# cage-challenge/cage-challenge-4

Hardware: AMD Instinct MI355X
Metric: agent-env steps/sec (5 blue agents x N envs) (higher is better)
Workload: dtype int32

## Files before the change

cage_challenge_4_amd/csrc/cc4_api.hip:

```cpp
#include "cc4_host.h"
#include "cc4_export.h"

static thread_local std::string g_create_err;
static std::mutex g_handles_mu;
static std::vector<cc4_handle*> g_handles;
std::atomic<int64_t> g_scoped_blocks{0};

__attribute__((constructor)) static void cc4_runtime_env() { setenv("GPU_MAX_HW_QUEUES", "16", 0); }

static int streams_run_concurrently(hipStream_t* st, int n) {
  if (n < 2) return 1;
  int khz = 100000, dev = 0;
  (void)hipGetDevice(&dev);
  (void)hipDeviceGetAttribute(&khz, hipDeviceAttributeWallClockRate, dev);
  if (khz <= 0) khz = 100000;
  const long long ticks = 300LL * khz / 1000;
  bool ok = true;
  double one = 0, all = 0;
  for (int pass = 0; pass < 2 && ok; ++pass) {
    const int m = pass ? n : 1;
    auto t0 = std::chrono::steady_clock::now();
    for (int i = 0; i < m; ++i) hipLaunchKernelGGL(k_spin, dim3(1), dim3(1), 0, st[i], ticks);
    for (int i = 0; i < m && ok; ++i) ok = hipStreamSynchronize(st[i]) == hipSuccess;
    const double us = std::chrono::duration<double, std::micro>(std::chrono::steady_clock::now() - t0).count();
    (pass ? all : one) = us;
  }
  return ok && all < 1.5 * (one > 300.0 ? one : 300.0);
}

static int policy_bits(const cc4_config& c) {
  return (c.red_policy & 3) | (c.green_policy ? GP_SLEEP_BIT : 0) | (c.green_policy == 2 ? GP_OPEN_BIT : 0) | (c.blue_policy ? BP_RANDOM_BIT : 0);
}
StepArgs step_args(const cc4_handle* h) {
  StepArgs a{};
  a.st = h->d_state; a.cold = h->d_cold;
  a.obs = h->d_obs; a.reward = h->d_reward; a.done = h->d_done; a.err = h->d_err;
  a.n = h->cfg.num_envs; a.autoreset = h->cfg.autoreset; a.steps = h->cfg.steps; a.rng_mode = h->cfg.rng_mode;
  a.policy = policy_bits(h->cfg);
  a.topo = (uint32_t)h->cfg.topology_seed;
  a.reset_ws = h->d_reset_ws;
  return a;
}
RunArgs run_args(const cc4_handle* h, int k, uint32_t t0, bool head) {
  RunArgs ra{};
  ra.progress = h->d_run; ra.slot_part = h->d_slot_part;
  ra.P = h->run_P; ra.K = k; ra.G = h->run_G; ra.t0 = t0;
  memcpy(ra.xcc_lo, h->xcc_lo, 8); memcpy(ra.xcc_n, h->xcc_n, 8);
  ra.thr = h->run_thr;
  ra.runs = head ? run_split_for_call(k, h->run_SA, h->run_SB, h->run_nB, h->run_single)
                 : run_split(k, h->run_SA, h->run_SB, h->run_nB, h->run_single);
  return ra;
}

void configure_groups(cc4_handle* h, int ng) {
  const int n = h->cfg.num_envs, cus = h->cus;
  if (ng < 1) ng = 1;
  if (ng > cc4_handle::MAX_GROUPS) ng = cc4_handle::MAX_GROUPS;
  if (ng > n) ng = n;
  h->ngroups = ng;
  for (int g = 0; g <= ng; ++g) h->glo[g] = (int)(((long long)n * g) / ng);
  const int gsize = (n + ng - 1) / ng;
  const int bpc = (gsize + cus - 1) / cus;
  const int bpc_all = (n + cus - 1) / cus;
  h->philox_minw = bpc <= 5 ? 1 : (bpc == 8 ? 8 : 7);
  if (ng > 1) h->philox_minw = bpc_all <= 6 ? 1 : 7;
  if (const char* v = getenv("CC4_PHILOX_MINW")) h->philox_minw = atoi(v);
  h->philox_lean = bpc > 8 || bpc_all > 13;
  if (const char* v = getenv("CC4_PHILOX_LEAN")) h->philox_lean = atoi(v) != 0;
}

int join_groups(cc4_handle* h) {
  if (h->rollout_k > 0 && !h->rollout_entering) { h->err = "a rollout is in flight on this handle: cc4_rollout_end first"; return -1; }
  if (h->ngroups > 1) {
    if (h->groups_busy) {
      for (int g = 1; g < h->ngroups; ++g) {
        HIPCHK(h, hipEventRecord(h->gev[g], h->gstream[g]));
        HIPCHK(h, hipStreamWaitEvent(h->stream, h->gev[g], 0));
      }
      h->groups_busy = false;
    }
    h->main_ahead = true;
    h->joined_between = true;
  }
  return 0;
}
int fork_groups(cc4_handle* h) {
  if (h->ngroups > 1 && h->main_ahead) {
    HIPCHK(h, hipEventRecord(h->mev, h->stream));
    for (int g = 1; g < h->ngroups; ++g) HIPCHK(h, hipStreamWaitEvent(h->gstream[g], h->mev, 0));
    h->main_ahead = false;
  }
  return 0;
}
int enter_refused(cc4_handle* h, const char* who, unsigned refuse) {
  if ((refuse & EN_NO_ROLLOUT) && h->rollout_k > 0) { h->err = std::string(who) + ": a rollout is in flight on this handle: cc4_rollout_end first"; return -2; }
  if ((refuse & EN_NO_COMM) && h->comm) { h->err = std::string(who) + ": not on a handle with a communicator"; return -2; }
  return 0;
}
int enter(cc4_handle* h, const char* who, unsigned refuse) {
  if (int rc = enter_refused(h, who, refuse)) return rc;
  HIPCHK(h, hipSetDevice(h->cfg.device_id));
  return join_groups(h) ? -1 : 0;
}
int copy_to_host(cc4_handle* h, const char* who, void* dst, const void* src, size_t bytes, hipMemcpyKind kind) {
  if (int rc = enter(h, who)) return rc;
  if (bytes) HIPCHK(h, hipMemcpyAsync(dst, src, bytes, kind, h->stream));
  HIPCHK(h, hipStreamSynchronize(h->stream));
  return 0;
}
int sync_all(cc4_handle* h) {
  for (int g = h->ngroups - 1; g >= 1; --g) if (h->groups_busy) HIPCHK(h, hipStreamSynchronize(h->gstream[g]));
  if (hipStreamQuery(h->stream) != hipSuccess) { (void)hipGetLastError(); HIPCHK(h, hipStreamSynchronize(h->stream)); }
  h->groups_busy = false;
  h->joined_between = true;
  return 0;
}

int wall_khz(cc4_handle* h) {
  if (h->khz <= 0) { int khz = 100000; (void)hipDeviceGetAttribute(&khz, hipDeviceAttributeWallClockRate, h->cfg.device_id); h->khz = khz > 0 ? khz : 100000; }
  return h->khz;
}
int ensure_watchdog_word(cc4_handle* h) {
  if (!h->h_xtimeout) {
// ... 91 lines not shown
const char* cc4_last_error(cc4_handle* h) { return h ? h->err.c_str() : g_create_err.c_str(); }
size_t cc4_state_bytes(void) { return sizeof(EnvState); }
int cc4_device_count(void) { int n = 0; return hipGetDeviceCount(&n) == hipSuccess ? n : 0; }
size_t cc4_algorithmic_bytes_per_env_step(void) {
  return 2 * sizeof(EnvState) + 4 * OBS_TOTAL + 4 * NBLUE + 4 + 1 + 4;
}
size_t cc4_hot_bytes(void) { return offsetof(EnvState, hd); }
const char* cc4_step_kernel(cc4_handle* h) {
  if (!h) return "";
  if (h->cfg.rng_mode != 1) return "k_step";
  return h->philox_lean ? "k_step_philox1" : "k_step_philox";
}

const char* cc4_run_kernel(cc4_handle* h) {
  if (!h) return "";
  const bool plain = (!h->comm || h->xchg_on) && !h->evlog_on && !h->ext_seen && !h->d_prof && !h->dbg_stop;
  if (plain && h->multistep) return h->multistep_minb == 8 ? "k_run_philox8" : "k_run_philox";
  if (plain && h->run1m) return "k_run_philox1m";
  if (plain && h->persist_state >= 0) return h->cfg.rng_mode == 0 ? "k_run_pcg" : (h->comm ? "k_run_philox1x" : "k_run_philox1");
  return cc4_step_kernel(h);
}
const char* cc4_run_kernel_for(cc4_handle* h, int32_t k) {
  if (!h) return "";
  if (h->persist_state == 0 && !h->run1m && !h->multistep && (!h->comm || h->xchg_on) && !h->evlog_on && !h->ext_seen && !h->d_prof && k >= h->persist_min_k && hipSetDevice(h->cfg.device_id) == hipSuccess) (void)persist_setup(h);
  const char* r = cc4_run_kernel(h);
  if (k < 2) return cc4_step_kernel(h);
  if (!h->multistep && !h->run1m && h->persist_state >= 0 && k < h->persist_min_k) return cc4_step_kernel(h);
  return r;
}

int cc4_create(const cc4_config* cfg, cc4_handle** out) {
  if (!cfg || !out || cfg->num_envs <= 0 || cfg->steps <= 0 || cfg->red_policy < 0 || cfg->red_policy > 3 ||
      cfg->green_policy < 0 || cfg->green_policy > 2 || cfg->blue_policy < 0 || cfg->blue_policy > 1 || cfg->rng_mode < 0 || cfg->rng_mode > 1) { g_create_err = "cc4_create: bad config"; return -2; }
  if (cfg->topology_seed != 0 && cfg->rng_mode != 1) { g_create_err = "cc4_create: topology_seed needs rng_mode 1 (the numpy stream draws scenario and dynamics from one generator)"; return -2; }
  int ndev = 0;
  hipError_t e = hipGetDeviceCount(&ndev);
  if (e != hipSuccess || ndev <= 0) {
    g_create_err = "cc4_create: no HIP device available (libcc4 has no CPU fallback)";
    return -3;
  }
  if (cfg->device_id < 0 || cfg->device_id >= ndev) { g_create_err = "cc4_create: device_id out of range"; return -2; }
  cc4_handle* h = new cc4_handle();
  h->cfg = *cfg;
  *out = h;
  { std::lock_guard<std::mutex> lk(g_handles_mu); g_handles.push_back(h); }
  if (const char* v = getenv("CC4_HOST_WAIT")) {
    static std::once_flag once;
    std::call_once(once, [v] {
      unsigned flags = hipDeviceScheduleAuto;
      if (!strcmp(v, "spin")) flags = hipDeviceScheduleSpin; else if (!strcmp(v, "yield")) flags = hipDeviceScheduleYield; else if (!strcmp(v, "block")) flags = hipDeviceScheduleBlockingSync;
      (void)hipSetDeviceFlags(flags);
      (void)hipGetLastError();
    });
  }
  HIPCHK(h, hipSetDevice(cfg->device_id));
  if (cc4_upload_pcg_tables() != hipSuccess) { h->err = "cc4_create: the numpy-stream kernel's jump table could not be uploaded"; return -1; }
  {
    hipDeviceProp_t prop;
    HIPCHK(h, hipGetDeviceProperties(&prop, cfg->device_id));
    h->cus = prop.multiProcessorCount > 0 ? prop.multiProcessorCount : 256;
  }
  {
    int ng = cfg->num_envs >= 1024 ? 3 : (cfg->num_envs >= 512 ? 2 : 1);
    h->auto_groups = getenv("CC4_GROUPS") == nullptr;
    if (const char* v = getenv("CC4_GROUPS")) ng = atoi(v);
    configure_groups(h, ng);
  }
  if (new_stream(h, &h->stream)) return -1;
  h->gstream[0] = h->stream;
  for (int g = 1; g < h->ngroups; ++g) {
    if (new_stream(h, &h->gstream[g]) || new_event(h, &h->gev[g], hipEventDisableTiming)) return -1;
  }
  if (new_event(h, &h->mev, hipEventDisableTiming) || new_event(h, &h->ev_wait, hipEventDisableTiming) || new_event(h, &h->ev_signal, hipEventDisableTiming)) return -1;
  if (h->auto_groups && h->ngroups == 3) {
    if (new_stream(h, &h->gstream[3])) return -1;
    if (streams_run_concurrently(h->gstream, 4)) {
      if (new_event(h, &h->gev[3], hipEventDisableTiming)) return -1;
      configure_groups(h, 4);
    } else release(h, &h->gstream[3]);
  }
  size_t n = (size_t)cfg->num_envs;
  h->cold_row = cold_row_bytes(cfg->steps);
  if (dev_alloc(h, &h->d_state, n * sizeof(EnvState)) || dev_alloc(h, &h->d_cold, n * h->cold_row)) return -1;
  if (dev_alloc(h, &h->d_reset_ws, cfg->rng_mode == 1 ? n * RESET_WS_WORDS * sizeof(uint32_t) : n * 128 * sizeof(uint64_t))) return -1;
  h->in_bytes = n * NBLUE * sizeof(int32_t) + n * NBLUE * MSG_LEN;
  h->small_io = cfg->num_envs <= cc4_handle::SMALL_IO_ENVS;
  if (const char* v = getenv("CC4_SMALL_IO")) h->small_io = h->small_io && atoi(v) != 0;
  if (h->small_io) {
    if (pin_alloc(h, &h->pin_in, h->in_bytes)) return -1;
    HIPCHK(h, hipHostGetDevicePointer(reinterpret_cast<void**>(&h->d_actions), h->pin_in, 0));
    memset(h->pin_in, 0, h->in_bytes);
  } else if (dev_alloc(h, &h->d_actions, h->in_bytes)) return -1;
  h->d_msgs = reinterpret_cast<uint8_t*>(h->d_actions) + n * NBLUE * sizeof(int32_t);
  if (dev_alloc(h, &h->d_seeds, n * sizeof(uint64_t)) || dev_alloc(h, &h->d_envmask, n)) return -1;
  h->out_bytes = n * OBS_TOTAL * sizeof(int32_t) + n * sizeof(float) + n * sizeof(uint32_t) + n;
  if (h->small_io) {
    if (pin_alloc(h, &h->pin_out, h->out_bytes)) return -1;
    HIPCHK(h, hipHostGetDevicePointer(reinterpret_cast<void**>(&h->d_obs), h->pin_out, 0));
  } else if (dev_alloc(h, &h->d_obs, h->out_bytes)) return -1;
  h->d_reward = reinterpret_cast<float*>(h->d_obs + n * OBS_TOTAL);
  h->d_err = reinterpret_cast<uint32_t*>(h->d_reward + n);
  h->d_done = reinterpret_cast<uint8_t*>(h->d_err + n);
  if (dev_alloc(h, &h->d_mask, n * MASK_TOTAL) || dev_alloc(h, &h->d_rng, n * 7 * sizeof(uint64_t))) return -1;
  if (dev_alloc(h, &h->d_claim, n * sizeof(uint32_t) + sizeof(uint32_t)) || dev_alloc(h, &h->d_mask_stale, n)) return -1;
  h->d_copy_fault = h->d_claim + n;
  HIPCHK(h, hipMemsetAsync(h->d_claim, 0, n * sizeof(uint32_t) + sizeof(uint32_t), h->stream));
  HIPCHK(h, hipMemsetAsync(h->d_mask_stale, 0, n, h->stream));
  HIPCHK(h, hipMemsetAsync(h->d_state, 0, n * sizeof(EnvState), h->stream));
  HIPCHK(h, hipMemsetAsync(h->d_cold, 0, n * h->cold_row, h->stream));
  HIPCHK(h, hipMemsetAsync(h->d_obs, 0, n * OBS_TOTAL * sizeof(int32_t), h->stream));
  HIPCHK(h, hipMemsetAsync(h->d_done, 0, n, h->stream));
  HIPCHK(h, hipMemsetAsync(h->d_err, 0, n * sizeof(uint32_t), h->stream));
  HIPCHK(h, hipStreamSynchronize(h->stream));
  if (choose_run_form(h, 0)) return -1;
  if (const char* v = getenv("CC4_PERSIST_MIN_K")) h->persist_min_k = atoi(v);
  if (const char* v = getenv("CC4_WHOLE_BATCH_STEPS")) h->whole_batch_steps = atoi(v) != 0;
  if (const char* v = getenv("CC4_PERSIST_VERIFY")) h->verify = atoi(v) != 0;
  if (const char* v = getenv("CC4_PERSIST_VERIFY_EVERY")) h->verify_every = atoi(v) > 0 ? atoi(v) : 0;
  return 0;
}

void cc4_destroy(cc4_handle* h) {
  if (!h) return;
  enq_pool_stop(h);
  (void)hipSetDevice(h->cfg.device_id);
  for (const OwnedList::Entry& e : h->own.entries) if (e.kind == OWN_STREAM && *e.field) (void)hipStreamSynchronize(static_cast<hipStream_t>(*e.field));
  if (h->comm) ncclCommDestroy(h->comm);
  if (h->shadow) { cc4_destroy(h->shadow); h->shadow = nullptr; (void)hipSetDevice(h->cfg.device_id); }
  h->own.release_all();
  { std::lock_guard<std::mutex> lk(g_handles_mu); g_handles.erase(std::remove(g_handles.begin(), g_handles.end(), h), g_handles.end()); }
  delete h;
}
int cc4_debug_live_resources(int64_t out[4]) {
  if (!out) return -2;
  out[OWN_DEVICE] = g_scoped_blocks.load(); out[OWN_PINNED] = out[OWN_EVENT] = out[OWN_STREAM] = 0;
  std::lock_guard<std::mutex> lk(g_handles_mu);
  for (const cc4_handle* h : g_handles) h->own.count_live(out);
  return 0;
}

static int reset_launch(cc4_handle* h, const uint64_t* d_seeds, const uint8_t* d_env_mask) {
  ResetArgs a{h->d_state, h->d_cold, d_seeds, d_env_mask, h->d_obs, h->d_reward,
              h->d_done, h->d_err, h->d_mask, h->cfg.num_envs, h->cfg.steps, h->cfg.rng_mode,
              policy_bits(h->cfg), (uint32_t)h->cfg.topology_seed,
              h->comm ? h->d_obs8[h->obs_buf] : nullptr};
  if (h->comm && h->gathers_issued > h->gathers_waited) { HIPCHK(h, hipStreamSynchronize(h->comm_stream)); h->gathers_waited = h->gathers_issued; }
  if (h->comm && h->obs8_from_slab >= 0) {
    const size_t row = (size_t)h->cfg.num_envs * OBS_PACKED;
    if (d_env_mask) HIPCHK(h, hipMemcpyAsync(h->d_obs8[h->obs_buf], h->d_xslab + (size_t)h->obs8_from_slab * row, row, hipMemcpyDeviceToDevice, h->stream));
    h->obs8_from_slab = -1;
  }
  hipLaunchKernelGGL(k_reset, dim3(h->cfg.num_envs), dim3(WAVE), 0, h->stream, a);
  HIPCHK(h, hipGetLastError());
  h->prev_valid = false;
  h->step_event_attached = false;
  return 0;
}
int cc4_reset(cc4_handle* h, const uint64_t* seeds, const uint8_t* env_mask) {
  if (int rc = enter(h, "cc4_reset")) return rc;
  size_t n = (size_t)h->cfg.num_envs;
  if (seeds) HIPCHK(h, hipMemcpyAsync(h->d_seeds, seeds, n * sizeof(uint64_t), hipMemcpyHostToDevice, h->stream));
  if (env_mask) HIPCHK(h, hipMemcpyAsync(h->d_envmask, env_mask, n, hipMemcpyHostToDevice, h->stream));
  if (int rc = reset_launch(h, seeds ? h->d_seeds : nullptr, env_mask ? h->d_envmask : nullptr)) return rc;
  HIPCHK(h, hipStreamSynchronize(h->stream));
  return 0;
}
int cc4_reset_device(cc4_handle* h, const uint64_t* d_seeds, const uint8_t* d_env_mask) {
// ... 505 lines not shown
```

cage_challenge_4_amd/csrc/cc4_api_debug.hip:

```cpp
#include "cc4_host.h"

int timeline_report(cc4_handle* h, int k, bool timed) {
  std::vector<unsigned long long> tl(4 * (size_t)h->run_grid);
  HIPCHK(h, hipMemcpy(tl.data(), h->d_timeline, tl.size() * sizeof(unsigned long long), hipMemcpyDeviceToHost));
  release(h, &h->d_timeline);
#ifdef CC4_BOUNDARY_PROF
  { double sA = 0, sB = 0, sC = 0, sD = 0, sn = 0, items = 0, busy_ticks = 0; int nw = 0; std::vector<double> per;
    bool head = false;
    for (int w = 0; w < h->run_grid; ++w) { const unsigned long long* t = &tl[4 * (size_t)w]; if (!(t[0] >> 63)) continue; head = true;
      const double n = (double)((t[0] >> 32) & 0x7FFFFFFFull); if (n <= 0) continue; ++nw;
      const double A = (double)(uint32_t)t[1], B = (double)(t[1] >> 32), C = (double)(uint32_t)t[2], D = (double)(t[2] >> 32);
      sA += A; sB += B; sC += C; sD += D; sn += n; items += (double)(uint32_t)t[3]; busy_ticks += (double)(uint32_t)t[0]; per.push_back((A + B + C + D) / n / 100.0); }
    if (head) {
      float ms = 0.f; if (timed) (void)hipEventElapsedTime(&ms, h->evs[0], h->evs[1]);
      std::sort(per.begin(), per.end());
      const size_t m = per.size();
      const RunSplit rs = h->last_runs;
      if (m) fprintf(stderr, "[cc4 boundary] k=%d runs SA=%d nA=%d SB=%d nB=%d nph=%d: %d waves with a boundary, %.0f boundaries (%.0f items); per boundary, mean us: stage-out drain + publish %.3f, pick %.3f, "
                      "progress wait + acquire %.3f, stage-in %.3f, all %.3f; per wave all: min %.3f / median %.3f / 90%% %.3f / max %.3f us; boundaries are %.2f %% of the waves' busy time "
                      "(first item's start to last item's end, mean %.1f us); kernel (events) %.1f us\n", k, rs.SA, rs.nA, rs.SB, rs.nB, rs.nph, nw, sn, items,
                      sA / sn / 100.0, sB / sn / 100.0, sC / sn / 100.0, sD / sn / 100.0, (sA + sB + sC + sD) / sn / 100.0, per[0], per[m / 2], per[m * 9 / 10], per[m - 1],
                      100.0 * (sA + sB + sC + sD) / busy_ticks, busy_ticks / nw / 100.0, ms * 1000.0);
      return 0;
    }
  }
#endif
  unsigned long long e0 = ~0ull, e1 = 0, f1 = 0, l0 = ~0ull, l1 = 0; double fs = 0, ls = 0, items = 0; int nw = 0, idle = 0;
  for (int w = 0; w < h->run_grid; ++w) { const unsigned long long* t = &tl[4 * (size_t)w]; if (!t[0]) continue; ++nw; e0 = t[0] < e0 ? t[0] : e0; e1 = t[0] > e1 ? t[0] : e1; if (!(uint32_t)t[3]) { ++idle; continue; } f1 = t[1] > f1 ? t[1] : f1; l0 = t[2] < l0 ? t[2] : l0; l1 = t[2] > l1 ? t[2] : l1; fs += (double)t[1]; ls += (double)t[2]; items += (double)(uint32_t)t[3]; }
  const int busy = nw - idle;
  float ms = 0.f; if (timed) (void)hipEventElapsedTime(&ms, h->evs[0], h->evs[1]);
  fprintf(stderr, "[cc4 timeline] k=%d: %d waves reported (%d without an item); entry spread %.1f us; first item starts: mean +%.1f us, last +%.1f us after the first entry; "
                  "last item ends: earliest +%.1f us, mean +%.1f us, latest +%.1f us; items per busy wave %.1f; kernel (events) %.1f us\n",
          k, nw, idle, (e1 - e0) / 100.0, busy ? (fs / busy - (double)e0) / 100.0 : 0.0, (f1 - e0) / 100.0, (l0 - e0) / 100.0, busy ? (ls / busy - (double)e0) / 100.0 : 0.0, (l1 - e0) / 100.0, busy ? items / busy : 0.0, ms * 1000.0);
  { std::map<int, std::pair<unsigned long long, double>> cu;
    for (int w = 0; w < h->run_grid; ++w) { const unsigned long long* t = &tl[4 * (size_t)w]; if (!t[0] || !(uint32_t)t[3]) continue; auto& c = cu[(int)((t[3] >> 32) - 1)]; if (t[2] > c.first) c.first = t[2]; c.second += (double)(uint32_t)t[3]; }
    std::vector<double> last, its; for (auto& kv : cu) { last.push_back((kv.second.first - e0) / 100.0); its.push_back(kv.second.second); }
    std::sort(last.begin(), last.end()); std::sort(its.begin(), its.end());
    if (!last.empty()) { const size_t m = last.size(); fprintf(stderr, "[cc4 timeline]   per CU (%zu): last wave dry at min %.1f / 10%% %.1f / median %.1f / 90%% %.1f / max %.1f us; items executed min %.0f / median %.0f / max %.0f\n", m,
                               last[0], last[m / 10], last[m / 2], last[m * 9 / 10], last[m - 1], its[0], its[m / 2], its[m - 1]); } }
  { double xs[8] = {0}, xi[8] = {0}; unsigned long long xl[8] = {0}, xf[8]; int xn[8] = {0}; for (int i = 0; i < 8; ++i) xf[i] = ~0ull;
    for (int w = 0; w < h->run_grid; ++w) { const unsigned long long* t = &tl[4 * (size_t)w]; if (!t[0] || !(uint32_t)t[3]) continue; const int xc = (int)(((t[3] >> 32) - 1) >> 8) & 7;
      xs[xc] += (double)t[2]; xi[xc] += (double)(uint32_t)t[3]; ++xn[xc]; if (t[2] > xl[xc]) xl[xc] = t[2]; if (t[2] < xf[xc]) xf[xc] = t[2]; }
    for (int i = 0; i < 8; ++i) if (xn[i]) fprintf(stderr, "[cc4 timeline]   XCD %d: %d busy waves, %.0f items; waves ran dry: earliest +%.1f, mean +%.1f, latest +%.1f us\n", i, xn[i], xi[i],
                                                  (xf[i] - e0) / 100.0, (xs[i] / xn[i] - (double)e0) / 100.0, (xl[i] - e0) / 100.0); }
  return 0;
}
void exchange_prof_report(int k, const std::chrono::steady_clock::time_point (&t)[6]) {
  static double xp[6] = {0}; static long xpn = 0;
  auto us = [](std::chrono::steady_clock::time_point a, std::chrono::steady_clock::time_point b) { return std::chrono::duration<double, std::micro>(b - a).count(); };
  xp[0] += us(t[0], t[1]); xp[1] += us(t[1], t[2]); xp[2] += us(t[2], t[3]); xp[3] += us(t[3], t[4]); xp[4] += us(t[4], t[5]); xp[5] += us(t[0], t[5]);
  if (++xpn % 200 == 0) {
    fprintf(stderr, "[cc4 exchange prof] k=%d, mean of 200 calls (us): begin %.1f, launch %.1f, enqueue of the chunks %.1f, wait for the kernel %.1f, then for the communication stream %.1f; call %.1f\n",
            k, xp[0] / 200, xp[1] / 200, xp[2] / 200, xp[3] / 200, xp[4] / 200, xp[5] / 200);
    for (double& v : xp) v = 0;
  }
}
int cc4_debug_rollout_state(cc4_handle* h, int64_t* out ) {
  if (!h->d_rcnt) { h->err = "cc4_debug_rollout_state: no rollout was begun on this handle"; return -2; }
  HIPCHK(h, hipSetDevice(h->cfg.device_id));
  std::vector<uint32_t> rd(32), cnt((size_t)h->run_P * RPG_MAX * cc4_handle::XRING);
  uint32_t fail = 0;
  HIPCHK(h, hipMemcpy(rd.data(), h->d_rready, rd.size() * 4, hipMemcpyDeviceToHost));
  HIPCHK(h, hipMemcpy(cnt.data(), h->d_rcnt, cnt.size() * 4, hipMemcpyDeviceToHost));
  HIPCHK(h, hipMemcpy(&fail, h->d_rfail, 4, hipMemcpyDeviceToHost));
  out[0] = fail; out[1] = *reinterpret_cast<volatile uint32_t*>(h->h_xtimeout);
  for (int g = 0; g < h->rpg; ++g) out[2 + g] = rd[g];
  for (int slot = 0; slot < 4; ++slot) for (int g = 0; g < h->rpg; ++g) {
    int64_t sum = 0;
    for (int p = 0; p < h->run_P; ++p) sum += cnt[((size_t)p * h->rpg + g) * cc4_handle::XRING + slot];
    out[6 + 4 * slot + g] = sum;
  }
  return 0;
}

int cc4_debug_profile(cc4_handle* h, int enable, unsigned long long* out) {
  if (int rc = enter(h, "cc4_debug_profile")) return rc;
  size_t bytes = (size_t)h->cfg.num_envs * PROF_SLOTS * sizeof(unsigned long long);
  if (enable && !h->d_prof) { if (dev_alloc(h, &h->d_prof, bytes)) return -1; HIPCHK(h, hipMemsetAsync(h->d_prof, 0, bytes, h->stream)); }
  if (out && h->d_prof) { HIPCHK(h, hipMemcpyAsync(out, h->d_prof, bytes, hipMemcpyDeviceToHost, h->stream)); HIPCHK(h, hipStreamSynchronize(h->stream)); }
  if (!enable) release(h, &h->d_prof);
  return 0;
}

int cc4_debug_stop_phase(cc4_handle* h, int phase) {
  if (join_groups(h)) return -1;
  if (phase < 0 || phase > 14 || !h->philox_lean) { h->err = "cc4_debug_stop_phase: phase 0..14, on a handle whose step kernel is k_step_philox1"; return -2; }
  h->dbg_stop = phase;
  return 0;
}

int cc4_debug_persist_base(cc4_handle* h, uint32_t base) {
  if (h->rollout_k > 0) { h->err = "cc4_debug_persist_base: a rollout is in flight on this handle"; return -2; }
  if (base > PROGRESS_CLEAR_AT) { char msg[64]; snprintf(msg, sizeof msg, "cc4_debug_persist_base: base 0 .. %#x", PROGRESS_CLEAR_AT); h->err = msg; return -2; }
  if (int rc = enter(h, "cc4_debug_persist_base")) return rc;
  if (h->persist_state == 0) { if (persist_setup(h)) return -1; }
  if (h->persist_state != 1) { h->err = "cc4_debug_persist_base: this handle has no persistent kernel"; return -2; }
  HIPCHK(h, hipMemsetD32Async(reinterpret_cast<hipDeviceptr_t>(h->d_run), (int)base, (size_t)h->cfg.num_envs, h->stream));
  HIPCHK(h, hipStreamSynchronize(h->stream));
  h->pool_base = base;
  return 0;
}
int cc4_debug_copy_from_device(cc4_handle* h, void* host_dst, const void* device_src, size_t bytes) {
  if (int rc = enter(h, "cc4_debug_copy_from_device")) return rc;
  HIPCHK(h, hipStreamSynchronize(h->stream));
  for (int g = 0; g < 4; ++g) if (h->gpolicy[g]) HIPCHK(h, hipStreamSynchronize(h->gpolicy[g]));
// ... 58 lines not shown
```

cage_challenge_4_amd/csrc/cc4_args.h:

```cpp
#pragma once
#include <hip/hip_runtime.h>

#include "../../include/cc4.h"
#include "cc4_engine.h"
#include "cc4_sched.h"

using namespace cc4;

static_assert(sizeof(EnvState) % 16 == 0 && offsetof(EnvState, hd) % 16 == 0, "EnvState rows are staged with 16-byte accesses");
constexpr int ROW_VEC = (int)(sizeof(EnvState) / 16);
constexpr int HOT_VEC = (int)(offsetof(EnvState, hd) / 16);
constexpr int WAVE = 64;
constexpr int OBS_PACKED = CC4_OBS_PACKED_BYTES;
static_assert(OBS_PACKED % 4 == 0 && OBS_PACKED * 4 >= OBS_TOTAL, "packed observation row: whole words, four values per byte");
constexpr int PROF_SLOTS = 128;

constexpr int cc4_handle_max_groups = 8;

#ifndef CC4_PERSIST_MINW
#define CC4_PERSIST_MINW 6
#endif
#ifndef CC4_LEAN_MINW
#define CC4_LEAN_MINW 1
#endif
#ifndef CC4_SMALL_MINW
#define CC4_SMALL_MINW 1
#endif
#ifndef CC4_PHILOX_BIG_MINW
#define CC4_PHILOX_BIG_MINW 7
#endif

struct StepArgs {
  EnvState* st; EnvCold* cold;
  const int32_t* actions; const uint8_t* msgs;
  int32_t* obs; float* reward; uint8_t* done; uint32_t* err;
  uint8_t* obs8;
  int32_t* rand_out;
  uint64_t rand_seed0; uint32_t rand_t;
  int n, autoreset, steps, rng_mode, policy;
  int full_obs;
  uint32_t topo;
  unsigned long long* prof;
  uint32_t* reset_ws;
  const ExtAct* ext;
  int e0;
  int act_sys;
  int dbg_stop;
};

struct XchgArgs {
  uint8_t* slab;
  uint32_t* gathered;
  uint32_t* timeout;
  int ring;
  long long wait_ticks;
  uint32_t* gcnt;
  uint32_t* timeout_host;
};

struct RunArgs {
  uint32_t* progress;
  const int32_t* slot_part;
  int P, K;
  int G;
  uint32_t t0;
  RunSplit runs;
  uint8_t xcc_lo[8], xcc_n[8];
  int thr;
  uint32_t* ticket;
  uint32_t* ticket_next;
  uint32_t base;
  unsigned long long* timeline;
  const uint32_t* act_ready;
  const int32_t* act;
  int PG;
  long long act_wait_ticks;
};
constexpr int TK_STRIDE = 32;
constexpr int CC4_SLOTS = 2048;
constexpr int RPG_MAX = 4;

struct PlanArgs {
  const int32_t* actions;
  const uint8_t* msgs;
  float* rewards;
  uint8_t* dones;
  uint8_t* obs_packed;
  uint32_t* err_or;
};
constexpr uint32_t PLAN_REGEN = 0x80000000u;

struct ResetArgs {
  EnvState* st; EnvCold* cold; const uint64_t* seeds; const uint8_t* env_mask;
  int32_t* obs; float* reward; uint8_t* done; uint32_t* err; uint8_t* mask;
  int n, steps, rng_mode, policy;
  uint32_t topo;
  uint8_t* obs8;
};

struct alignas(16) SlotHdr {
  uint32_t magic, version;
  int32_t steps, rng_mode;
  uint32_t claim;
  uint32_t pad[11];
};
static_assert(sizeof(SlotHdr) == 64, "64-byte slot header");
constexpr uint32_t SLOT_MAGIC = 0x45344343u;
constexpr uint32_t SLOT_VERSION = (1u << 24) | (uint32_t)((sizeof(EnvState) + sizeof(EnvCold)) & 0xFFFFFFu);
constexpr size_t SLOT_OUT_BYTES = 192;
CC4_HD size_t slot_cold_off() { return sizeof(SlotHdr) + sizeof(EnvState); }
CC4_HD size_t slot_out_off(size_t cold_row) { return slot_cold_off() + ((cold_row + 63) & ~(size_t)63); }
CC4_HD size_t slot_bytes(size_t cold_row) { return slot_out_off(cold_row) + SLOT_OUT_BYTES; }
static_assert(OBS_PACKED + 12 <= (int)SLOT_OUT_BYTES && sizeof(SlotHdr) % 64 == 0 && sizeof(EnvState) % 64 == 0, "slot layout");
enum : uint32_t { CF_RANGE = CC4_COPY_RANGE, CF_DUP_DST = CC4_COPY_DUP_DST, CF_SRC_IS_DST = CC4_COPY_SRC_IS_DST, CF_SLOT_EMPTY = CC4_COPY_SLOT_EMPTY,
                  CF_SLOT_CONFIG = CC4_COPY_SLOT_CONFIG };
CC4_HD uint32_t slot_hdr_fault(const SlotHdr* hdr, int steps, int rng_mode) {
  if (hdr->magic != SLOT_MAGIC || hdr->version != SLOT_VERSION) return CF_SLOT_EMPTY;
  return hdr->steps != steps || hdr->rng_mode != rng_mode ? CF_SLOT_CONFIG : 0u;
}
struct CopyArgs {
  EnvState* st; EnvCold* cold; size_t cold_row;
  int32_t* obs; float* reward; uint8_t* done; uint32_t* err; uint8_t* mask; uint8_t* mask_stale;
  uint32_t* claim;
  const uint8_t* src_bank; uint8_t* dst_bank; size_t slot;
  const int32_t* src; const int32_t* dst; const uint64_t* seeds;
  int count, n, src_cap, dst_cap, steps, rng_mode, evlog_on;
// ... 56 lines not shown
```

cage_challenge_4_amd/csrc/cc4_engine.h:

```cpp
#pragma once
#include "cc4_state.h"
#include "cc4_tables.h"

namespace cc4 {

struct Ctx { EnvState* s; EnvCold* c; Rng* r; HostDyn* hd; StepWork* w; unsigned long long* prof = nullptr;
             unsigned long long* aprof = nullptr; EvLog* lg = nullptr; const uint64_t* gpre = nullptr;
             const ExtAct* ext = nullptr; };

#if defined(__HIP_DEVICE_COMPILE__)
#define CC4_TICK(x, i) do { if ((x).prof) { unsigned long long _t = clock64(); (x).prof[(i)] += _t - (x).prof[15]; (x).prof[15] = _t; } } while (0)
#define CC4_TICK0(x) do { if ((x).prof) (x).prof[15] = clock64(); } while (0)
#define CC4_AT0(x) unsigned long long _at = (x).aprof ? clock64() : 0
#define CC4_AT(x, k) do { if ((x).aprof) { unsigned long long _n = clock64(); (x).aprof[(k)] += _n - _at; _at = _n; } } while (0)
#if defined(CC4_FINE)
#define CC4_FT0(x, r) unsigned long long _ft = ((x).aprof && (r) == 0) ? clock64() : 0
#define CC4_FT(x, r, k) do { if ((x).aprof && (r) == 0) { unsigned long long _n = clock64(); (x).aprof[88 + (k)] += _n - _ft; _ft = _n; } } while (0)
#else
#define CC4_FT0(x, r) do { } while (0)
#define CC4_FT(x, r, k) do { } while (0)
#endif
#else
#define CC4_FT0(x, r) do { } while (0)
#define CC4_FT(x, r, k) do { } while (0)
// ... 524 lines not shown
  if (flags & OE_SYSHN) bit_set(a.as_hn, host);
  if (subnet_known) a.h.as_subnet |= (uint16_t)(1u << h_subnet(host));
  uint8_t want = (uint8_t)(key_ip ? OE_KEY_IP : 0);
  uint32_t* has = a.obs_has[key_ip ? 1 : 0];
  if (bit_get(has, host)) {
    for (int i = 0; i < a.h.nobs; ++i)
      if (a.obs[i].host == host && (a.obs[i].flags & OE_KEY_IP) == want) { a.obs[i].flags |= (uint8_t)flags; return; }
  }
  bit_set(has, host);
  if (a.h.nobs >= MAX_OBS) { set_err(x, E_OBS_OVERFLOW); return; }
  a.obs[a.h.nobs].host = (uint8_t)host;
  a.obs[a.h.nobs].flags = (uint8_t)(flags | want);
  a.h.nobs++;
}
CC4_HD void obs_first(Ctx x, int r, int success, int atype, int ahost, int aarg) {
  RedAgent& a = x.s->red[r];
  if (a.h.obs_success != 0) return;
  const uint32_t v = hdr_obs_word((uint32_t)success, (uint32_t)atype, (uint32_t)ahost, (uint32_t)aarg);
  __builtin_memcpy(__builtin_assume_aligned(reinterpret_cast<char*>(&a.h) + offsetof(RedHdr, obs_success), 4), &v, 4);
}

CC4_HD int path_to_root(int h, uint8_t* out) {
  int n = 0;
  out[n++] = (uint8_t)h;
  if (h == H_INTERNET) return n;
  int s = h_subnet(h);
  if (!h_is_router(h)) out[n++] = (uint8_t)h_make(s, 0);
  while (true) {
    int p = router_parent(s);
    if (p == S_INT) { out[n++] = (uint8_t)H_INTERNET; break; }
    out[n++] = (uint8_t)h_make(p, 0);
    s = p;
  }
  return n;
}
CC4_HD int route(int src, int dst, uint8_t* work) {
  uint8_t* a = work; uint8_t* b = work + 6; uint8_t* out = work + 12;
  int na = path_to_root(src, a), nb = path_to_root(dst, b);
  while (na >= 2 && nb >= 2 && a[na - 2] == b[nb - 2]) { na--; nb--; }
  int n = 0;
  for (int i = 0; i < na; ++i) out[n++] = a[i];
  for (int i = nb - 2; i >= 0; --i) out[n++] = b[i];
  return n;
}

CC4_HD int gen_pid(Ctx x, uint32_t* used) {
  while (true) {
    int pid = rng_range(x.r, 1000, 10000);
    if (!bit_get(used, pid - 1000)) { bit_set(used, pid - 1000); return pid; }
  }
}
CC4_HD int start_session_proc(Ctx x, int h, int kind) {
  HostDyn& st = x.hd[h];
  int mx = 0;
  for (int i = 0; i < st.nproc; ++i) if (st.procs[i].pid > mx) mx = st.procs[i].pid;
  int pid = mx + 1 + (int)rng_below(x.r, 9);
  st.procs[st.nproc].pid = (uint16_t)pid; st.procs[st.nproc].kind = (uint8_t)kind; st.procs[st.nproc].flags = 0;
  st.nproc++;
  return pid;
}
CC4_HD void host_backup(Ctx x, int h, int ip_octet) {
  const HostDyn& d = x.hd[h];
  HostStatic st;
  for (int i = 0; i < 8; ++i) st.procs[i] = d.procs[i];
  for (int i = 0; i < 5; ++i) st.svcs[i] = d.svcs[i];
  st.nproc = (uint8_t)d.nproc; st.nsvc = (uint8_t)hd_nsvc(d); st.exists = (uint8_t)(1 | ((d.gtmp & 1) << 1)); st.ip_octet = (uint8_t)ip_octet;
  if (d.nproc > PIN - 1 || hd_nsvc(d) > 5) set_err(x, E_PROC_OVERFLOW);
  __builtin_memcpy(&x.c->hs[h], &st, sizeof(HostStatic));
}
CC4_HD void host_restore(Ctx x, int h) {
  hd_touch(x, h);
  HostDyn& d = x.hd[h];
  HostStatic st;
  __builtin_memcpy(&st, &x.c->hs[h], sizeof(HostStatic));
  for (int i = 0; i < 8; ++i) d.procs[i] = st.procs[i];
  for (int i = 0; i < 5; ++i) d.svcs[i] = st.svcs[i];
  d.nproc = st.nproc; d.gtmp = 0; d.nsf = st.nsvc;
  x.s->hev[h] = 0;
  eph_clear(x, h);
  pend_drop_host(x, h);
}

struct ResetCarry { uint64_t env_key; };
enum : int { RESET_WS_SEEN = 0, RESET_WS_DUP = 288, RESET_WS_HOSTS = 576, RESET_WS_WORDS = 584 };

CC4_HD void reset_zero(EnvState* s, HostDyn* hd, EnvCold* c, int t, int nt) {
  static_assert(offsetof(EnvState, rng) == 0, "the generator leads the row");
  uint32_t* w = (uint32_t*)s;
  for (size_t i = sizeof(Rng) / 4 + (size_t)t; i < offsetof(EnvState, hd) / 4; i += (size_t)nt) w[i] = i == PA_WORD ? w[i] & PA_WORD_MASK : 0;
  uint32_t* hw = (uint32_t*)hd;
  for (size_t i = (size_t)t; i < sizeof(HostDyn) * MAXH / 4; i += (size_t)nt) hw[i] = 0;
  uint32_t* b = (uint32_t*)c->hs;
  for (size_t i = (size_t)t; i < sizeof(c->hs) / 4; i += (size_t)nt) b[i] = 0;
}
static_assert(sizeof(RSess) * RS_POOL >= 4 * 282, "the idle session pool holds the 9000-bit pid set of the generation");
CC4_HD uint32_t* reset_used_set(EnvState* s) { return reinterpret_cast<uint32_t*>(s->spool); }
CC4_HD void reset_used_clear(EnvState* s, int t, int nt) { uint32_t* u = reset_used_set(s); for (int i = t; i < 282; i += nt) u[i] = 0; }
template <int RNG_MODE>
CC4_HD void reset_gen_host(Ctx x, int h) {
  EnvState* s = x.s;
  if (!bit_get(s->exists, h)) return;
  if (RNG_MODE == 1) rng_set_stream(x.r, ST_GEN_HOST + (uint32_t)h);
  HostDyn& st = x.hd[h];
  st.gtmp = (uint8_t)rng_below(x.r, 2);
  if (h_is_router(h)) return;
  int n = 0;
  auto put = [&](int kind, int pid) {
    st.svcs[n].kind = (uint8_t)kind; st.svcs[n].pid = (uint16_t)pid; st.svcs[n].st = (uint8_t)(SV_ACTIVE | 5);
    st.procs[n].kind = (uint8_t)kind; st.procs[n].pid = (uint16_t)pid; st.procs[n].flags = 0;
    n++;
  };
  auto pid = [&]() { return RNG_MODE == 1 ? rng_range(x.r, 1000, 10000) : gen_pid(x, reset_used_set(s)); };
  put(K_SSHD, pid());
  int sub = h_subnet(h);
  if (sub == S_OZA || sub == S_OZB) put(K_OT, pid());
  int p_apache = pid(), p_mysql = pid(), p_smtp = pid();
  int n_add = (int)rng_below(x.r, 4);
  uint32_t left = 7;
  for (int k = 0; k < n_add; ++k) {
    int o = nth_bit(left, (int)rng_below(x.r, (uint32_t)popc32(left)));
    left &= ~(1u << o);
    put(o == 0 ? K_APACHE : (o == 1 ? K_MYSQL : K_SMTP), o == 0 ? p_apache : (o == 1 ? p_mysql : p_smtp));
  }
  for (int i = 0; i < n; ++i) (void)rng_random(x.r);
  hd_set_nsvc(st, n); st.nproc = (uint16_t)n;
  if (RNG_MODE == 1) { st.procs[5].pid = (uint16_t)p_apache; st.procs[6].pid = (uint16_t)p_mysql; st.svcs[6].pid = (uint16_t)p_smtp; }
}
struct ResetHostLater { CC4_HD void operator()(Ctx, int) const {} };
struct ResetHostNow { CC4_HD void operator()(Ctx x, int h) const { reset_gen_host<0>(x, h); } };
CC4_HD void reset_mission_phases(EnvState* s, int steps) {
  int q = steps / 3, rem = steps % 3;
  s->steps = steps;
  s->phase_len[0] = q + (rem >= 1 ? 1 : 0); s->phase_len[1] = q + (rem == 2 ? 1 : 0); s->phase_len[2] = q;
}
template <int RNG_MODE, typename HostHook>
CC4_HD ResetCarry reset_topology(Ctx x, uint64_t seed, int steps, bool continue_stream, int policy, uint32_t topo_seed, uint32_t* ws,
                                 bool rng_is_copy, HostHook host_placed) {
  EnvState* s = x.s;
  if (!continue_stream) rng_seed(&s->rng, seed, (uint32_t)RNG_MODE);
  s->rng_mode = (uint8_t)RNG_MODE;
  s->policy = (uint8_t)policy_at_reset(s, policy);
  rng_begin_episode(x.r);
  ResetCarry k; k.env_key = x.r->s_lo;
  if (RNG_MODE == 1 && topo_seed) x.r->s_lo = (uint64_t)topo_seed;
  reset_mission_phases(s, steps);
  if (RNG_MODE == 1) for (int i = 0; i < RESET_WS_WORDS; ++i) ws[i] = 0;
  {
    uint32_t* avail = x.w->scratch;
    for (int i = 0; i < 8; ++i) avail[i] = 0xFFFFFFFFu;
    int n = 256;
    for (int sn = 0; sn < NSUB; ++sn) {
      int v = nth_set(avail, 8, (int)rng_below(x.r, (uint32_t)n));
      s->cidr_octet[sn] = (uint8_t)v;
      bit_clr(avail, v);
      n--;
    }
  }
  for (int sn = 0; sn < NSUB; ++sn) {
    uint32_t* ips = x.w->scratch;
    for (int i = 0; i < 8; ++i) ips[i] = 0xFFFFFFFFu;
    ips[0] &= ~1u; ips[7] &= 0x7FFFFFFFu;
    int n = 254;
    auto place = [&](int h, int v) {
      bit_clr(ips, v); n--; bit_set(s->exists, h); x.hd[h].procs[PIN - 1].pid = (uint16_t)v;
      host_placed(x, h);
    };
    if (sn == S_INT) { place(H_INTERNET, nth_set(ips, 8, (int)rng_below(x.r, (uint32_t)n))); continue; }
    place(h_make(sn, 0), nth_set(ips, 8, (int)rng_below(x.r, (uint32_t)n)));
    int nu = 3 + (int)rng_below(x.r, 8);
    for (int i = 0; i < nu; ++i) place(h_make(sn, 1 + i), nth_set(ips, 8, (int)rng_below(x.r, (uint32_t)n)));
    int ns = 1 + (int)rng_below(x.r, 6);
    for (int i = 0; i < ns; ++i) place(h_make(sn, 11 + i), last_set(ips, 8));
    s->n_users[sn] = (uint8_t)nu; s->n_servers[sn] = (uint8_t)ns;
  }
  if (RNG_MODE == 1 && rng_is_copy) s->rng = *x.r;
  return k;
}
CC4_HD void reset_pid_serial(Ctx x, uint32_t* used) {
  EnvState* s = x.s;
  for (int h = 0; h < MAXH; ++h) {
    if (!bit_get(s->exists, h) || h_is_router(h)) continue;
    HostDyn& st = x.hd[h];
    const int n = hd_nsvc(st);
    const int sub = h_subnet(h);
    const int nfix = (sub == S_OZA || sub == S_OZB) ? 2 : 1;
    Rng t; bool forked = false;
    auto settle = [&](int v0, bool* moved) {
      int v = v0 - 1000;
      *moved = false;
      while (bit_get(used, v)) {
        if (!forked) { rng_fork(&t, x.r, ST_GEN_REDRAW + (uint32_t)h); forked = true; }
        v = (int)rng_below(&t, 9000);
        *moved = true;
      }
      bit_set(used, v);
      return v + 1000;
    };
    for (int i = 0; i < nfix; ++i) {
      bool moved;
      const int v = settle(st.svcs[i].pid, &moved);
      if (moved) { st.svcs[i].pid = (uint16_t)v; st.procs[i].pid = (uint16_t)v; }
    }
    for (int k = 0; k < 3; ++k) {
      const int kind = k == 0 ? K_APACHE : (k == 1 ? K_MYSQL : K_SMTP);
      const int v0 = k == 0 ? st.procs[5].pid : (k == 1 ? st.procs[6].pid : st.svcs[6].pid);
      bool moved;
      const int v = settle(v0, &moved);
      if (moved) for (int i = nfix; i < n; ++i) if (st.svcs[i].kind == kind) { st.svcs[i].pid = (uint16_t)v; st.procs[i].pid = (uint16_t)v; }
    }
    st.procs[5].pid = 0; st.procs[6].pid = 0; st.svcs[6].pid = 0;
  }
}
CC4_HD void reset_agents(Ctx x) {
  EnvState* s = x.s;
  for (int b = 0; b < NBLUE; ++b) {
    int nsub = blue_nsub(b);
    (void)rng_below(x.r, (uint32_t)nsub);
    int cnt = 0;
    for (int i = 0; i < nsub; ++i) { int sn = blue_subnet_alloc(b, i); cnt += 1 + s->n_users[sn] + s->n_servers[sn]; }
    int c = (int)rng_below(x.r, (uint32_t)cnt);
    int ph = -1;
    for (int i = 0; i < nsub && ph < 0; ++i) {
      int sn = blue_subnet_alloc(b, i), nu = s->n_users[sn], ns = s->n_servers[sn];
      if (c < 1 + nu) ph = h_make(sn, c);
      else if (c < 1 + nu + ns) ph = h_make(sn, 11 + (c - 1 - nu));
      else c -= 1 + nu + ns;
    }
    s->blue[b].parent_host = (uint8_t)ph;
  }
  {
    int g = 0;
    for (int sn = 0; sn < NSUB - 1; ++sn) for (int i = 0; i < s->n_users[sn]; ++i) s->green_host[g++] = (uint8_t)h_make(sn, 1 + i);
    s->n_green = (uint8_t)g;
  }
  for (int r = 0; r < NRED; ++r) {
    int sn = red_subnet_alloc(r, (int)rng_below(x.r, (uint32_t)red_nsub(r)));
    int c = (int)rng_below(x.r, (uint32_t)(s->n_users[sn] + s->n_servers[sn]));
    s->red[r].h.start_host = (uint8_t)(c < s->n_users[sn] ? h_make(sn, 1 + c) : h_make(sn, 11 + (c - s->n_users[sn])));
    s->red[r].h.new_sess_host = 0xFF;
  }
}
CC4_HD void reset_seal_host(Ctx x, int h) {
  host_backup(x, h, x.hd[h].procs[PIN - 1].pid);
  x.hd[h].procs[PIN - 1].pid = 0; x.hd[h].gtmp = 0;
}
CC4_HD void reset_host_sessions(Ctx x, int h) {
  EnvState* s = x.s;
  if (!bit_get(s->exists, h)) return;
  rng_set_stream(x.r, ST_GEN_SESS + (uint32_t)h);
  if (blue_of_subnet(h_subnet(h)) >= 0) (void)start_session_proc(x, h, K_SESS_BLUE);
  if (h != H_INTERNET && h_is_user(h)) (void)start_session_proc(x, h, K_SESS_GREEN);
  if (h == s->red[0].h.start_host) (void)start_session_proc(x, h, K_SESS_RED);
  reset_seal_host(x, h);
}
CC4_HD void reset_sessions_agent_order(Ctx x) {
  EnvState* s = x.s;
  for (int b = 0; b < NBLUE; ++b) {
    int ph = s->blue[b].parent_host;
    (void)start_session_proc(x, ph, K_SESS_BLUE);
    for (int i = 0; i < blue_nsub(b); ++i) {
      int sn = blue_subnet_alloc(b, i);
      for (int sl = 0; sl < SLOTS; ++sl) {
        int h = h_make(sn, sl);
        if (!bit_get(s->exists, h) || h == ph) continue;
        (void)start_session_proc(x, h, K_SESS_BLUE);
      }
    }
  }
  for (int g = 0; g < s->n_green; ++g) (void)start_session_proc(x, s->green_host[g], K_SESS_GREEN);
  (void)start_session_proc(x, s->red[0].h.start_host, K_SESS_RED);
}
CC4_HD void reset_seal_all_hosts(Ctx x) {
  EnvState* s = x.s;
  for (int h = 0; h < MAXH; ++h) {
    if (bit_get(s->exists, h)) reset_seal_host(x, h);
    eph_clear(x, h);
  }
  s->npend = 0;
}
CC4_HD void reset_finish(Ctx x, ResetCarry k, int steps, uint32_t topo_seed, bool rng_is_copy) {
  EnvState* s = x.s;
  {
    const HostDyn& d = x.hd[s->red[0].h.start_host];
    int red0_pid = 0;
    for (int i = 0; i < d.nproc; ++i) if (d.procs[i].kind == K_SESS_RED) red0_pid = d.procs[i].pid;
    (void)rs_add(x, 0, s->red[0].h.start_host, red0_pid, RS_ABSTRACT | RS_ORIG);
    s->red[0].h.active = 1;
  }
  for (int r = 0; r < NRED; ++r) {
    RedAgent& a = s->red[r];
    int h = a.h.start_host;
    bit_set(a.as_ip, h); bit_set(a.as_hn, h); a.h.as_subnet |= (uint16_t)(1u << h_subnet(h));
    if (r == 0) {
      as_know_sid(x, 0, 0);
      obs_put(x, 0, false, h, OE_SESS | OE_IFACE | OE_SYSHN, true);
      obs_first(x, 0, T_UNKNOWN, RA_NONE, 0, 0);
    }
    a.h.exec_type = RA_SLEEP;
  }
  s->done = (uint8_t)(0 >= steps - 1);
  s->n_actions = NBLUE + s->n_green + NRED;
  x.c->rwd = RewardRec{};
  if (topo_seed) x.r->s_lo = k.env_key;
  if (rng_is_copy) s->rng = *x.r;
  rng_park(&s->rng);
}
CC4_HD void env_reset_counter_mode(Ctx x, uint64_t seed, int steps, bool continue_stream, int policy, uint32_t topo_seed, uint32_t* ws,
                                   bool rng_is_copy) {
  reset_zero(x.s, x.hd, x.c, 0, 1);
  ResetCarry k = reset_topology<1>(x, seed, steps, continue_stream, policy, topo_seed, ws, rng_is_copy, ResetHostLater{});
  {
    Rng t; rng_fork(&t, x.r, ST_GEN_HOST);
    Ctx xh = x; xh.r = &t;
    for (int h = 0; h < MAXH; ++h) reset_gen_host<1>(xh, h);
  }
  reset_pid_serial(x, reset_used_set(x.s));
  reset_used_clear(x.s, 0, 1);
  reset_agents(x);
  {
    Rng t; rng_fork(&t, x.r, ST_GEN_SESS);
    Ctx xh = x; xh.r = &t;
    for (int h = 0; h < MAXH; ++h) reset_host_sessions(xh, h);
  }
  reset_finish(x, k, steps, topo_seed, rng_is_copy);
}
CC4_HD void env_reset_numpy_stream(Ctx x, uint64_t seed, int steps, bool continue_stream, int policy, bool rng_is_copy) {
  reset_zero(x.s, x.hd, x.c, 0, 1);
  ResetCarry k = reset_topology<0>(x, seed, steps, continue_stream, policy, 0, nullptr, rng_is_copy, ResetHostNow{});
  reset_used_clear(x.s, 0, 1);
  reset_agents(x);
  reset_sessions_agent_order(x);
  reset_seal_all_hosts(x);
  reset_finish(x, k, steps, 0, rng_is_copy);
}

CC4_HD void env_reset(Ctx x, uint64_t seed, int rng_mode, int steps, bool continue_stream, int policy = 0, uint32_t topo_seed = 0,
                      uint32_t* ws = nullptr, bool rng_is_copy = false) {
  if (rng_mode == 1) env_reset_counter_mode(x, seed, steps, continue_stream, policy, topo_seed, ws, rng_is_copy);
  else env_reset_numpy_stream(x, seed, steps, continue_stream, policy, rng_is_copy);
}

enum : int { BLUE_RAW_ACTION = 0x10000 };
CC4_HD constexpr uint32_t blue_slot_shape(int b, int idx) {
  const int nsub = blue_nsub(b), nh = ZONE_HOSTS * nsub, nc = 8 * nsub;
  int t = BA_SLEEP, j = 0;
  if (idx < 0 || idx >= 4 * nh + 2 + 2 * nc) return (uint32_t)BA_SLEEP;
  if (idx < nh) { t = BA_ANALYSE; j = idx; }
  else if (idx == nh) return (uint32_t)BA_MONITOR;
  else if (idx < 2 * nh + 1) { t = BA_REMOVE; j = idx - nh - 1; }
  else if (idx < 3 * nh + 1) { t = BA_RESTORE; j = idx - 2 * nh - 1; }
  else if (idx == 3 * nh + 1) return (uint32_t)BA_SLEEP;
  else if (idx < 3 * nh + 2 + nc) { t = BA_ALLOW; j = idx - 3 * nh - 2; }
  else if (idx < 3 * nh + 2 + 2 * nc) { t = BA_BLOCK; j = idx - 3 * nh - 2 - nc; }
  else { t = BA_DECOY; j = idx - 3 * nh - 2 - 2 * nc; }
  if (t == BA_ALLOW || t == BA_BLOCK) {
    const int dst = blue_subnet_sorted(b, j / 8), k = j % 8;
    int src = 0, c = 0;
    for (int i = 0; i < NSUB; ++i) { const int sn = sorted_subnet(i); if (sn == dst) continue; if (c == k) { src = sn; break; } c++; }
    return (uint32_t)t | ((uint32_t)dst << 8) | ((uint32_t)src << 16);
  }
  const int sn = blue_subnet_sorted(b, j / ZONE_HOSTS), hs = j % ZONE_HOSTS;
  const int h = hs < MAX_SERVERS ? h_make(sn, 11 + hs) : h_make(sn, 1 + (hs - MAX_SERVERS));
  return (uint32_t)t | ((uint32_t)h << 8);
}
#if defined(__HIP_DEVICE_COMPILE__)
struct BlueSlotTab { uint32_t v[NBLUE][ACT_LONG]; };
constexpr BlueSlotTab make_blue_slot_tab() {
  BlueSlotTab t{};
  for (int b = 0; b < NBLUE; ++b) for (int i = 0; i < ACT_LONG; ++i) t.v[b][i] = blue_slot_shape(b, i);
  return t;
}
static __device__ const BlueSlotTab blue_slot_tab = make_blue_slot_tab();
__device__ __forceinline__ uint32_t blue_slot(int b, int idx) { return blue_slot_tab.v[b][idx]; }
#else
CC4_HD uint32_t blue_slot(int b, int idx) { return blue_slot_shape(b, idx); }
#endif
CC4_HD Act blue_decode(const EnvState* s, int b, int idx) {
  Act a; a.type = BA_SLEEP; a.host = 0; a.arg = 0; a.ticks = 1; a.sid = 0; a.busy = 0;
  int nsub = blue_nsub(b), nh = ZONE_HOSTS * nsub, nc = 8 * nsub;
  int total = 4 * nh + 2 + 2 * nc;
  if (idx >= BLUE_RAW_ACTION) {
    const int t = (idx >> 8) & 0xF, h = idx & 0xFF;
    if (t == BA_BLOCK || t == BA_ALLOW) {
      const int to = h & 0xF, from = h >> 4;
      if (to >= NSUB || from >= NSUB) return a;
      a.type = (uint8_t)t; a.host = (uint8_t)to; a.arg = (uint8_t)from;
      return a;
    }
    if (t == BA_MONITOR) { a.type = BA_MONITOR; return a; }
    if (t < BA_ANALYSE || t > BA_DECOY || h >= H_INTERNET || !bit_get(s->exists, h) || blue_of_subnet(h_subnet(h)) != b) return a;
    a.type = (uint8_t)t; a.host = (uint8_t)h;
    return a;
  }
  if (idx < 0 || idx >= total) return a;
  const uint32_t sh = blue_slot(b, idx);
  const int t = (int)(sh & 0xFF), h = (int)((sh >> 8) & 0xFF);
  if (t == BA_SLEEP) return a;
  if (t == BA_MONITOR) { a.type = BA_MONITOR; return a; }
  if (t == BA_ALLOW || t == BA_BLOCK) { a.type = (uint8_t)t; a.host = (uint8_t)h; a.arg = (uint8_t)(sh >> 16); return a; }
// ... 1621 lines not shown
```

cage_challenge_4_amd/csrc/cc4_host.h:

```cpp
#pragma once
#include <hip/hip_runtime.h>
#include <hip/hip_ext.h>
#include <rccl/rccl.h>
#include <stdio.h>
#include <stdlib.h>
#include <string.h>
#include <string>
#include <chrono>
#include <vector>
#include <deque>
#include <map>
#include <algorithm>
#include <thread>
#include <mutex>
#include <condition_variable>
#include <atomic>

#include "../../include/cc4_debug.h"
#include "cc4_args.h"
#include "cc4_kernel_decls.h"
#include "cc4_export.h"
#include "cc4_digest.h"
#include "cc4_owned.h"
#define CC4_HOST __attribute__((visibility("hidden")))

inline void free_device(void* p) { (void)hipFree(p); }
inline void free_pinned(void* p) { (void)hipHostFree(p); }
inline void free_event(void* p) { (void)hipEventDestroy(static_cast<hipEvent_t>(p)); }
inline void free_stream(void* p) { (void)hipStreamDestroy(static_cast<hipStream_t>(p)); }

struct cc4_handle {
  cc4_config cfg;
  OwnedList own{{free_device, free_pinned, free_event, free_stream}, {}};
  hipStream_t stream = nullptr;
  EnvState* d_state = nullptr; EnvCold* d_cold = nullptr;
  size_t cold_row = 0;
  int32_t* d_actions = nullptr; uint8_t* d_msgs = nullptr; uint64_t* d_seeds = nullptr; uint8_t* d_envmask = nullptr;
  int32_t* d_obs = nullptr; float* d_reward = nullptr; uint8_t* d_done = nullptr; uint32_t* d_err = nullptr;
  uint8_t* d_mask = nullptr; uint64_t* d_rng = nullptr;
  size_t out_bytes = 0, in_bytes = 0;
  uint8_t* pin_out = nullptr; uint8_t* pin_in = nullptr;
  static constexpr int SMALL_IO_ENVS = 16;
  bool small_io = false;
  bool keep_prev = false, prev_valid = false;
  EnvState* d_prev_state = nullptr; EnvCold* d_prev_cold = nullptr; uint8_t* d_prev_out = nullptr;
  const int32_t* prev_actions = nullptr; const uint8_t* prev_msgs = nullptr; bool prev_full_obs = false, prev_ext = false;
  static constexpr int OBS_RING = 8, OBS_WAIT_EVERY = 4;
  static constexpr int MAX_GROUPS = cc4_handle_max_groups;
  uint8_t* d_obs8[OBS_RING] = {};
  uint8_t* d_all_obs8[OBS_RING] = {};
  long long gather_seq[OBS_RING] = {};
  long long gathers_issued = 0, gathers_waited = 0;
  hipEvent_t tev_start[cc4_handle_max_groups] = {}, tev_stop[cc4_handle_max_groups] = {};
  long long comm_delay_ticks = 0;
  long long gather_stalls = 0;
  long long stat_steps = 0; double stat_launch_us = 0, stat_gather_us = 0;
  hipStream_t comm_stream = nullptr;
  hipEvent_t ev_step[OBS_RING][MAX_GROUPS] = {}, ev_comm[OBS_RING] = {};
  int obs_buf = 0;
  int gather_buf = -1;
  bool step_event_attached = false;
  int ngroups = 1;
  int cus = 256;
  int glo[MAX_GROUPS + 1] = {};
  hipStream_t gstream[MAX_GROUPS] = {};
  hipEvent_t gev[MAX_GROUPS] = {};
  hipEvent_t mev = nullptr;
  hipEvent_t ev_wait = nullptr, ev_signal = nullptr;
  bool auto_groups = true;
  bool groups_busy = false;
  bool joined_between = false;
  bool main_ahead = false;
  unsigned long long* d_prof = nullptr;
  int dbg_stop = 0;
  uint32_t* d_reset_ws = nullptr;
  uint8_t* d_unpacked = nullptr;
  int evlog_on = 0;
  uint32_t* d_run = nullptr;
  int32_t* d_slot_part = nullptr;
  unsigned long long* d_timeline = nullptr;
  size_t run_words = 0;
  int run_P = 0, run_grid = 0;
  int run_G = 0;
  uint8_t xcc_lo[8] = {0}, xcc_n[8] = {0};
  int run_thr = 16;
  uint32_t* d_pool = nullptr;
  int run_SA = 0, run_SB = 1, run_nB = 0, run_single = 0;
  RunSplit last_runs{};
  uint32_t pool_base = 0;
  int pool_parity = 0;
  int persist_state = -1;
  bool whole_batch_steps = true;
  int run_margin = 0;
  static constexpr int XRING = 32;
  bool xchg_on = false;
  int xchg_chunk = 8;
  uint8_t* d_xslab = nullptr;
  uint8_t* d_xall = nullptr;
  int khz = 0;
  int32_t* d_ract = nullptr;
  uint32_t* d_rready = nullptr;
  uint32_t* d_rcnt = nullptr;
  uint32_t* d_rfail = nullptr;
  hipStream_t policy_stream = nullptr;
  hipStream_t gpolicy[4] = {nullptr, nullptr, nullptr, nullptr};
  hipEvent_t rev = nullptr;
  int rollout_k = 0;
  bool rollout_entering = false;
  int rollout_watchdog_ms = 2000;
  int rollout_margin = 1;
  int rpg = 4;
  int obs8_from_slab = -1;
  uint32_t* d_xflags = nullptr;
  uint32_t* d_xgcnt = nullptr;
  uint32_t* h_xtimeout = nullptr;
  uint32_t* d_xtimeout = nullptr;
  int xflags_clean = 0;
  hipEvent_t xev = nullptr;
  long long xchg_calls = 0, xchg_timeouts = 0;
  int xchg_watchdog_ms = 2000;
  uint8_t* last_gathered = nullptr;
  uint8_t* d_xlog = nullptr;
  int xlog_cap = 0, xlog_n = 0;
  bool persist_refused = false;
  bool verify = false, is_shadow = false;
  int verify_every = 1024;
  uint64_t persist_calls = 0;
  cc4_handle* shadow = nullptr;
  uint64_t* d_digest = nullptr;
  uint32_t* d_plan_err = nullptr;
  long long verify_calls = 0, verify_mismatches = 0;
  struct VerifyPlant { int32_t part = -1, env = 0, step = 0; int64_t offset = 0; } plant;
  int persist_min_k = 10;
  struct EnqPool* pool = nullptr;
  bool enq_threads = false;
  bool run1m = false;
  int multistep_minb = 5;
  bool multistep = false;
  ExtAct* d_ext = nullptr;
  bool ext_seen = false, ext_dirty = false;
  bool ext_submitted = false, terms_on = false;
  bool ext_green_dirty = true;
  std::vector<ExtAct> h_ext;
  bool full_obs_next = true;
  uint32_t full_obs_gmask = 0;
  bool philox_lean = false;
  int philox_minw = 1;
  ncclComm_t comm = nullptr; int rank = 0, world = 1;
  uint32_t* d_claim = nullptr; uint32_t* d_copy_fault = nullptr; uint8_t* d_mask_stale = nullptr;
  int32_t* d_copy_idx = nullptr; uint64_t* d_copy_seeds = nullptr;
  int8_t* d_pol = nullptr;
  std::deque<hipEvent_t> evs;
  std::string err;
};

#define HIPCHK(h, call)                                                                        \
  do {                                                                                         \
    hipError_t _e = (call);                                                                    \
// ... 79 lines not shown
```

cage_challenge_4_amd/csrc/cc4_k_misc.hip:

```cpp
#include "cc4_persist.h"
#include "cc4_kernel_decls.h"
#include "cc4_digest.h"

__global__ __launch_bounds__(WAVE) void k_xchg_gate(uint32_t* gcnt, int ring, int groups, int n, int P, int k_lo, int k_hi, long long ticks, uint32_t* fail, int max_naps) {
  const int t = (int)threadIdx.x, steps = k_hi - k_lo + 1;
  const long long t0 = wall_clock64();
  for (int i = t; i < groups * steps; i += (int)blockDim.x) {
    const int g = i / steps, k = k_lo + i % steps;
    const int size = P > 0 ? part_episodes(n, P, g) : xchg_group32_size(n, g);
    if (size <= 0) continue;
    uint32_t* c = gcnt + (size_t)g * (size_t)ring + (k % ring);
    int naps = 1;
    while (__hip_atomic_load(c, __ATOMIC_RELAXED, __HIP_MEMORY_SCOPE_AGENT) < (uint32_t)size) {
      for (int q = 0; q < naps; ++q) __builtin_amdgcn_s_sleep(127);
      if (naps < max_naps) naps <<= 1;
      if (wall_clock64() - t0 > ticks) { __hip_atomic_store(fail, 1u, __ATOMIC_RELAXED, __HIP_MEMORY_SCOPE_SYSTEM); break; }
    }
    __hip_atomic_store(c, 0u, __ATOMIC_RELAXED, __HIP_MEMORY_SCOPE_AGENT);
  }
}
__global__ __launch_bounds__(WAVE) void k_discover(int32_t* count, long long ticks) {
  if (threadIdx.x == 0) {
    atomicAdd(&count[cu_slot()], 1);
    const long long t0 = wall_clock64();
    while (wall_clock64() - t0 < ticks) __builtin_amdgcn_s_sleep(32);
  }
}
__global__ __launch_bounds__(WAVE) void k_reset(ResetArgs a) {
  __shared__ uint8_t obs_lds[OBS_TOTAL + 2];
  __shared__ uint8_t mask_lds[MASK_TOTAL + 2];
  __shared__ StepWork work;
  const int e = blockIdx.x, lane = threadIdx.x;
  if (e >= a.n) return;
  if (a.env_mask && !a.env_mask[e]) return;
  EnvCold* const cold_e = cold_at(a.cold, (size_t)e, cold_row_bytes(a.steps));
  EnvState* s = a.st + e;
  HostDyn* const hd = s->hd;
  for (int i = lane; i < (int)(sizeof(StepWork) / 4); i += WAVE) reinterpret_cast<uint32_t*>(&work)[i] = 0;
  __syncthreads();
  if (a.rng_mode == 1) {
    __shared__ uint32_t ws[RESET_WS_WORDS];
    reset_counter_mode_block<WAVE, false>(s, hd, cold_e, &work, lane, ws, a.seeds ? a.seeds[e] : 0, a.seeds == nullptr, a.steps, a.policy, a.topo);
    __syncthreads();
  } else if (lane == 0) {
    Ctx x{s, cold_e, &s->rng, hd, &work};
    env_reset(x, a.seeds ? a.seeds[e] : 0, 0, a.steps, a.seeds == nullptr, a.policy, a.topo);
  }
  if (lane == 0) {
    env_flat_obs<uint8_t>(s, obs_lds);
    blue_action_mask(s, mask_lds);
    a.reward[e] = 0.f; a.done[e] = s->done; a.err[e] = s->err;
  }
  __syncthreads();
  int32_t* o = a.obs + (size_t)e * OBS_TOTAL;
  for (int i = lane; i < OBS_TOTAL; i += WAVE) o[i] = obs_lds[i];
  uint8_t* m = a.mask + (size_t)e * MASK_TOTAL;
  for (int i = lane; i < MASK_TOTAL; i += WAVE) m[i] = mask_lds[i];
  if (a.obs8) store_packed_row(a.obs8 + (size_t)e * OBS_PACKED, obs_lds, lane, WAVE);
}

__global__ void k_random_actions(int32_t* actions, int n, uint64_t seed0, uint32_t t, int e0) {
  int i = e0 * NBLUE + blockIdx.x * blockDim.x + threadIdx.x;
  if (i >= n * NBLUE) return;
  int e = i / NBLUE, b = i % NBLUE;
  actions[i] = random_blue_action(seed0, t, e, b);
}

__global__ void k_spin(long long cycles) {
  const long long t0 = wall_clock64();
  while (wall_clock64() - t0 < cycles) __builtin_amdgcn_s_sleep(32);
}

__global__ void k_unpack_obs(const uint8_t* __restrict__ packed, uint8_t* __restrict__ out, int rows) {
  const int r = blockIdx.x, j = threadIdx.x;
  if (r >= rows || j >= OBS_PACKED) return;
  const uint32_t b = packed[(size_t)r * OBS_PACKED + j];
  uint8_t* o = out + (size_t)r * OBS_TOTAL + 4 * j;
#pragma unroll
  for (int k = 0; k < 4; ++k) if (4 * j + k < OBS_TOTAL) o[k] = (uint8_t)((b >> (2 * k)) & 3u);
}

template <int DT> __device__ __forceinline__ uint32_t policy_half_bits(int x) {
  constexpr uint64_t tab = DT == 1 ? 0x420040003C000000ull : 0x404040003F800000ull;
  return (uint32_t)(tab >> (16 * (x & 3))) & 0xFFFFu;
}
template <int DT> __device__ __forceinline__ void policy_obs_put(void* out, size_t i, int4 v) {
  if constexpr (DT == 0) {
    reinterpret_cast<uint32_t*>(out)[i] = (uint32_t)(v.x & 0xFF) | (uint32_t)(v.y & 0xFF) << 8 | (uint32_t)(v.z & 0xFF) << 16 | (uint32_t)(v.w & 0xFF) << 24;
  } else if constexpr (DT == 3) {
    reinterpret_cast<float4*>(out)[i] = make_float4((float)v.x, (float)v.y, (float)v.z, (float)v.w);
  } else {
    reinterpret_cast<uint2*>(out)[i] = make_uint2(policy_half_bits<DT>(v.x) | policy_half_bits<DT>(v.y) << 16, policy_half_bits<DT>(v.z) | policy_half_bits<DT>(v.w) << 16);
  }
}
template <int DT> __device__ __forceinline__ void policy_obs_part(const int32_t* __restrict__ obs, void* __restrict__ out, size_t total, size_t i0, size_t stride) {
  const size_t nv = total / 4;
  const int4* __restrict__ src = reinterpret_cast<const int4*>(obs);
  for (size_t i = i0; i < nv; i += stride) policy_obs_put<DT>(out, i, src[i]);
  if (i0 == 0) {
    for (size_t j = 4 * nv; j < total; ++j) {
      const int x = obs[j];
      if constexpr (DT == 0) reinterpret_cast<uint8_t*>(out)[j] = (uint8_t)x;
      else if constexpr (DT == 3) reinterpret_cast<float*>(out)[j] = (float)x;
      else reinterpret_cast<uint16_t*>(out)[j] = (uint16_t)policy_half_bits<DT>(x);
    }
  }
}
__global__ __launch_bounds__(256) void k_policy_outputs(const EnvState* __restrict__ st, const int32_t* __restrict__ obs, const float* __restrict__ reward,
                                                        const uint8_t* __restrict__ done, const uint32_t* __restrict__ err, int n, int ep_blocks, int dtype,
                                                        void* __restrict__ out_obs, uint8_t* __restrict__ out_mask, float* __restrict__ out_reward,
                                                        uint8_t* __restrict__ out_done, int32_t* __restrict__ out_err, uint8_t* __restrict__ mask_stale) {
  if ((int)blockIdx.x < ep_blocks) {
    const int e = (int)(blockIdx.x * blockDim.x + threadIdx.x), lane = (int)threadIdx.x & (WAVE - 1);
    bool regen = false;
    if (e < n) {
      out_reward[e] = reward[e]; out_done[e] = done[e]; out_err[e] = (int32_t)err[e];
      regen = st[e].step_count == 0;
      if (mask_stale[e]) { regen = true; mask_stale[e] = 0; }
    }
    unsigned long long todo = __ballot(regen);
    while (todo) {
      const int k = __ffsll(todo) - 1;
      todo &= todo - 1;
      const int er = e - lane + k;
      const EnvState* s = st + er;
// ... 129 lines not shown
```

cage_challenge_4_amd/csrc/cc4_k_pcg.hip:

```cpp
#include "cc4_kernels.h"
#include "cc4_persist.h"

struct PcgJump { uint64_t a_hi, a_lo, b_hi, b_lo; };
__device__ PcgJump g_pcg_jump[WAVE + 1];
__device__ __forceinline__ uint64_t bcast64(uint64_t v) {
  return (uint64_t)(uint32_t)__builtin_amdgcn_readfirstlane((int)(uint32_t)v) | ((uint64_t)(uint32_t)__builtin_amdgcn_readfirstlane((int)(uint32_t)(v >> 32)) << 32);
}
__device__ __forceinline__ uint32_t rdlane(uint32_t v, int j) { return (uint32_t)__builtin_amdgcn_readlane((int)v, j); }
__device__ __forceinline__ uint64_t lane64(uint64_t v, int src) {
  return (uint64_t)(uint32_t)__builtin_amdgcn_readlane((int)(uint32_t)v, src) | ((uint64_t)(uint32_t)__builtin_amdgcn_readlane((int)(uint32_t)(v >> 32), src) << 32);
}
__device__ __forceinline__ void pcg_ahead(const PcgJump& J, uint64_t s_hi, uint64_t s_lo, uint64_t i_hi, uint64_t i_lo, uint64_t* o_hi, uint64_t* o_lo) {
  const uint64_t p_lo = J.a_lo * s_lo, p_hi = __umul64hi(J.a_lo, s_lo) + J.a_hi * s_lo + J.a_lo * s_hi;
  const uint64_t q_lo = J.b_lo * i_lo, q_hi = __umul64hi(J.b_lo, i_lo) + J.b_hi * i_lo + J.b_lo * i_hi;
  const uint64_t lo = p_lo + q_lo;
  *o_lo = lo; *o_hi = p_hi + q_hi + (lo < p_lo ? 1ull : 0ull);
}
__device__ __forceinline__ uint64_t pcg_output(uint64_t hi, uint64_t lo) {
  const uint64_t v = hi ^ lo; const uint32_t rot = (uint32_t)(hi >> 58);
  return (v >> rot) | (v << ((64u - rot) & 63u));
}
__device__ __forceinline__ bool wave_green_policy(Rng& rl, int n, uint8_t* green_act, int lane) {
  const uint64_t s_hi = bcast64(rl.s_hi), s_lo = bcast64(rl.s_lo), i_hi = bcast64(rl.inc_hi), i_lo = bcast64(rl.inc_lo);
  const uint32_t has32 = (uint32_t)__builtin_amdgcn_readfirstlane((int)rl.has32), u32 = (uint32_t)__builtin_amdgcn_readfirstlane((int)rl.u32);
// ... 191 lines not shown
      int i = 0; uint32_t n32 = 0; bool hard = false;
      auto fetch = [&]() { uint64_t v = f[0]; if (i == 1) v = f[1]; if (i == 2) v = f[2]; if (i == 3) v = f[3]; if (i >= 4) v = f[4]; ++i; return v; };
      auto take32 = [&]() { ++n32; if (has) { has = 0; return buf; } const uint64_t o = fetch(); buf = (uint32_t)(o >> 32); q_new = pos + i - 1; has = 1; return (uint32_t)o; };
      auto below = [&](uint32_t n) { if (n <= 1) return 0u; const uint64_t m = (uint64_t)take32() * n; if ((uint32_t)m < n) hard = true; return (uint32_t)(m >> 32); };
      uint32_t r = GR_VALID;
      if (my_act == 0) {
        const int c = (int)below((uint32_t)(pre >> 56));
        int sn;
        const int dest = green_as_dest(pre, c, &sn);
        const uint32_t p = below(EPH_RANGE);
        r |= GR_EPH | ((uint32_t)dest << 8) | (p << 16);
        if ((my_blk >> sn) & 1u) r |= GR_FAIL | GR_CONN;
        else if ((fetch() >> 11) <= P01_FLOOR) r |= GR_CONN;
      } else if (!lw_am) r |= GR_FAIL;
      else {
        const int c = nth_bit8(lw_am, (int)below((uint32_t)popc32(lw_am)));
        const int rel = (int)((pre >> (8 * c)) & 0x7F) * 20;
        if ((int)below(100) >= rel) r |= GR_FAIL;
        else {
          if ((fetch() >> 11) <= P01_FLOOR) { const uint32_t p = below(EPH_RANGE); r |= GR_EPH | GR_PROC | (gh << 8) | (p << 16); }
          if ((fetch() >> 11) <= P01_FLOOR) r |= GR_PHISH;
        }
      }
      if (hard || pos + 5 > GW_OUT || ((uint32_t)i | (n32 << 16)) != d_cur || q_new != q_cur) r |= GR_HARD;
      rec = r;
    }
    if (stuck) rec |= GR_HARD;
    const int cnt = (ng - g0) < WAVE ? (ng - g0) : WAVE;
    int kend = cnt;
    enum { R_NEXT, R_HARD, R_PHISH } reason = R_NEXT;
    const uint64_t m_hard = __ballot((rec & GR_HARD) != 0), m_phish = __ballot((rec & GR_PHISH) != 0);
    if (m_hard) { const int k = __ffsll((unsigned long long)m_hard) - 1; if (k < kend) { kend = k; reason = R_HARD; } }
    if (m_phish) { const int k = __ffsll((unsigned long long)m_phish) - 1; if (k < kend) { kend = k + 1; reason = R_PHISH; } }
    const unsigned long long t1 = gstat ? clock64() : 0;
    const uint32_t eh = (rec >> 8) & 0xFFu, ep = (rec >> 16) & 0x3FFFu;
    bool coll = false;
    const bool has_port = lane < kend && (rec & GR_EPH);
    if (has_port) coll = eph_test_and_set(x.c, (int)eh, ep);
    const uint64_t cm = __ballot(coll);
    if (cm) {
      const int kc = __ffsll((unsigned long long)cm) - 1;
      if (has_port && !coll && lane >= kc) __hip_atomic_fetch_and(&x.c->eph[eh][ep >> 5], ~(1u << (ep & 31)), __ATOMIC_RELAXED, __HIP_MEMORY_SCOPE_WORKGROUP);
      kend = kc; reason = R_HARD;
    }
    if (lane < kend && (rec & GR_VALID)) {
      if (rec & GR_CONN) ev_or(x, (int)eh, EV_CUR_CONN);
      if (rec & GR_PROC) ev_or(x, (int)eh, EV_CUR_PROC);
      if (rec & GR_FAIL) __hip_atomic_fetch_add(&s->brm, reward_table(s->phase, h_subnet((int)gh), my_act == 0 ? RW_ASF : RW_LWF), __ATOMIC_RELAXED, __HIP_MEMORY_SCOPE_WORKGROUP);
    }
    int pos_e = 0; uint32_t has_e = has0, u_e = u0;
    if (kend > 0) {
      const uint32_t ie = rdlane(inc, kend - 1);
      const int qe = (int)rdlane((uint32_t)qinc, kend - 1);
      pos_e = (int)(ie & 0xFFFFu); has_e = (has0 + (ie >> 16)) & 1u;
      if (qe >= 0) u_e = (uint32_t)(win[qe] >> 32);
    }
    uint64_t n_hi = s_hi, n_lo = s_lo;
    if (pos_e > 0) {
      const int j = (pos_e - 1) & 63;
      n_hi = lane64(h0, j); n_lo = lane64(l0, j);
      if (pos_e > WAVE) { n_hi = lane64(h1, j); n_lo = lane64(l1, j); }
    }
    const unsigned long long t2 = gstat ? clock64() : 0;
    const int gend = g0 + kend;
    if (lane == 0) {
      rl.s_hi = n_hi; rl.s_lo = n_lo; rl.has32 = has_e; rl.u32 = u_e; rl.ndraw += (uint32_t)pos_e;
      if (reason == R_PHISH) phishing(x, s->green_host[gend - 1]);
      else if (reason == R_HARD) {
        s->brm += step_green_exec(x, gend);
        if (bit_get(x.w->phish_mask, gend)) { bit_clr(x.w->phish_mask, gend); phishing(x, s->green_host[gend]); }
      }
    }
    if (gstat && lane == 0) {
      gstat[0] += 1; gstat[1] += reason == R_PHISH; gstat[2] += m_hard != 0; gstat[3] += cm != 0;
      gstat[4] += t1 - t0; gstat[5] += t2 - t1; gstat[6] += clock64() - t2; gstat[7] += rounds + 1;
    }
    g0 = reason == R_HARD ? gend + 1 : gend;
  }
}

template <bool LOG>
__device__ __forceinline__ void pcg_body(StepArgs a, const int e, const int lane, const bool first, const bool last) {
  extern __shared__ uint4 lds[];
  uint64_t* const win_mem = reinterpret_cast<uint64_t*>(a.reset_ws) + (size_t)e * GW_OUT;
  if constexpr (!LOG) a.prof = nullptr;
  __shared__ int ok_lds;
  __shared__ StepWork work;
  EnvCold* const cold_e = cold_at(a.cold, (size_t)e, cold_row_bytes(a.steps));
  unsigned long long t_begin = a.prof ? clock64() : 0;
  const uint4* src = reinterpret_cast<const uint4*>(a.st + e);
  if (first) stage_in<HOT_VEC>(lds, src, lane);
  for (int i = lane; i < (int)(sizeof(StepWork) / 4); i += WAVE) reinterpret_cast<uint32_t*>(&work)[i] = 0;
  __syncthreads();
  EnvState* s = reinterpret_cast<EnvState*>(lds);
  HostDyn* const hd = a.st[e].hd;
  __shared__ unsigned long long prof_lds[LOG ? 16 : 1];
  unsigned long long* prof = a.prof ? prof_lds : nullptr;
  if (prof && lane < 16) prof_lds[lane] = 0;
  Rng rl = s->rng;
  rl.mode = 0;
  rl.pad = 0;
  Ctx x{s, cold_e, &rl, hd, &work, lane == 0 ? prof : nullptr};
  x.lg = (LOG && cold_e->evlog.enabled) ? &cold_e->evlog : nullptr;
  const ExtAct* const xt = (LOG && a.ext) ? a.ext + (size_t)e * EXT_PER_ENV : nullptr;
  x.ext = xt;
  if (prof && lane == 0) prof[11] += clock64() - t_begin;
  const bool do_reset = a.autoreset && s->done;
  const bool step_ok = !do_reset && step_phase_of(s->step_count, s->phase_len[0], s->phase_len[1], s->phase_len[2]) >= 0;
  if (lane == 0) {
    ok_lds = step_ok ? 1 : 0;
    if (do_reset) {
      env_reset(x, 0, 0, a.steps, true, a.policy, a.topo);
    } else {
      CC4_TICK0(x);
      (void)step_phase(x, false);
      CC4_TICK(x, 0);
      if (step_ok) rng_policy_swap(x, false);
      if (step_ok && (s->policy & BP_RANDOM_BIT))
        for (int b = 0; b < NBLUE; ++b) {
          int32_t act = a.actions ? a.actions[e * NBLUE + b] : -1;
          if (a.rand_out) { act = random_blue_action(a.rand_seed0, a.rand_t, e, b); a.rand_out[e * NBLUE + b] = act; }
          step_blue_submit(x, b, act);
        }
    }
  } else if (step_ok && lane <= NBLUE && !(s->policy & BP_RANDOM_BIT)) {
    const int b = lane - 1;
    int32_t act = a.actions ? a.actions[e * NBLUE + b] : -1;
    if (a.rand_out) { act = random_blue_action(a.rand_seed0, a.rand_t, e, b); a.rand_out[e * NBLUE + b] = act; }
    Ctx xb{s, cold_e, &rl, hd, &work};
    xb.ext = xt;
    step_blue_submit(xb, b, act);
  }
  __syncthreads();
  if (ok_lds) {
    bool drawn = false;
    if (!(s->policy & GP_SLEEP_BIT) && !xt) drawn = wave_green_policy(rl, s->n_green, work.green_act, lane);
    if (lane < NRED) { Ctx xo{s, cold_e, &rl, hd, &work}; xo.ext = xt; step_red_observe(xo, lane); }
    __syncthreads();
    if (lane == 0) {
      if (!drawn) for (int g = 0; g < s->n_green; ++g) step_green_policy(x, g);
      CC4_TICK(x, 1);
      for (int r = 0; r < NRED; ++r) s->n_actions -= step_red_policy_tick(x, r, (s->policy & 3) != RP_RANDOM);
      rng_policy_swap(x, true);
      CC4_TICK(x, 2);
      for (int b = 0; b < NBLUE; ++b) step_tick_blue(x, b);
      CC4_TICK(x, 3);
    }
    __syncthreads();
    wave_shuffle_consume(rl, s->n_actions, lane);
    if (lane == 0) { CC4_TICK(x, 4); step_blue_exec(x, true); }
  }
  __syncthreads();
  if (ok_lds) {
    if constexpr (!LOG) wave_green_exec(x, rl, win_mem, lane, nullptr);
    else {
      __shared__ uint64_t gpre_lds[MAXG];
      for (int g = lane; g < s->n_green; g += WAVE) { const int act = work.green_act[g]; if (act < 2) gpre_lds[g] = green_prepare(x, g, act); }
      __syncthreads();
      if (lane == 0) {
        Ctx xg = x; xg.gpre = gpre_lds;
        for (int g = 0; g < s->n_green; ++g) {
          s->brm += step_green_exec(xg, g);
          if (bit_get(work.phish_mask, g)) { bit_clr(work.phish_mask, g); phishing(x, s->green_host[g]); }
        }
      }
    }
    if (lane == 0) {
// ... 69 lines not shown
```

cage_challenge_4_amd/csrc/cc4_k_philox4.hip:

```cpp
#include "cc4_kernels.h"

constexpr int PW = 4;
static_assert(PW >= 4 && PW <= 8, "waves 0/1 run the two green action lists, waves PW-2 and PW-1 the green draws, wave PW-1 the blue submissions");
constexpr int PT = PW * WAVE;

__device__ __forceinline__ void stage_in_n(uint4* __restrict__ lds, const uint4* __restrict__ src, int tid) {
  constexpr int U = (ROW_VEC / PT) < 6 ? (ROW_VEC / PT) : 6;
  int i = tid;
  for (; i + (U - 1) * PT < ROW_VEC; i += U * PT) {
    uint4 v[U];
#pragma unroll
    for (int u = 0; u < U; ++u) v[u] = src[i + u * PT];
#pragma unroll
    for (int u = 0; u < U; ++u) lds[i + u * PT] = v[u];
  }
  for (; i < ROW_VEC; i += PT) lds[i] = src[i];
}

constexpr int HD_V0 = (int)((offsetof(EnvState, hd) + 15) / 16);
constexpr int HD_CHUNKS = (int)(((offsetof(EnvState, hd) + sizeof(HostDyn) * MAXH) / 16 - HD_V0) / 64);
constexpr int HD_V1 = HD_V0 + 64 * HD_CHUNKS;
__device__ __forceinline__ void dma_chunk(const uint4* gsrc_lane, uint4* lds_chunk_base) {
  const uint32_t dst = __builtin_amdgcn_readfirstlane((uint32_t)(uintptr_t)(__attribute__((address_space(3))) void*)lds_chunk_base);
  uint32_t keep;
  asm volatile("s_mov_b32 %0, m0\n\ts_mov_b32 m0, %2\n\ts_nop 0\n\tglobal_load_lds_dwordx4 %1, off\n\ts_mov_b32 m0, %0"
               : "=&s"(keep) : "v"(gsrc_lane), "s"(dst) : "memory");
}
__device__ __forceinline__ void dma_wait() { asm volatile("s_waitcnt vmcnt(0)" ::: "memory"); }

template <bool LOG, bool RUN = false>
__device__ __forceinline__ void philox4_body(StepArgs a, const int run_flags = 0, const int tid_in = -1, uint8_t* const obs_row = nullptr) {
  extern __shared__ uint4 lds[];
  __shared__ int conflict_lds;
  __shared__ alignas(16) uint32_t reset_ws[RESET_WS_WORDS];
  static_assert(RESET_WS_WORDS >= 4 * (MAXG + NRED + NBLUE), "one 16-byte block per green agent, red action stream and blue action stream");
  __shared__ int glist_n[2][2];
  __shared__ StepWork work;
  __shared__ uint8_t obs_bytes_own[OBS_TOTAL + 2];
  uint8_t* const obs_bytes = obs_row ? obs_row : obs_bytes_own;
  __shared__ uint8_t glist[2][2][MAXG];
  __shared__ unsigned long long prof_lds[16];
  const int e = a.e0 + (int)blockIdx.x, tid = tid_in >= 0 ? tid_in : (int)threadIdx.x, lane = tid & 63;
  const int wave = __builtin_amdgcn_readfirstlane(tid >> 6);
  if (e >= a.n) return;
  EnvCold* const cold_e = cold_at(a.cold, (size_t)e, cold_row_bytes(a.steps));
  unsigned long long t_begin = a.prof ? clock64() : 0;
  const uint4* src = reinterpret_cast<const uint4*>(a.st + e);
  constexpr int NA = HD_V0 + ROW_VEC - HD_V1;
  constexpr int NA_U = (NA + PT - 1) / PT;
  if (!RUN || !(run_flags & 1)) {
    {
      uint4 va[NA_U];
#pragma unroll
      for (int u = 0; u < NA_U; ++u) { int k = tid + u * PT; k = k < NA ? k : NA - 1; int i = k < HD_V0 ? k : k - HD_V0 + HD_V1; va[u] = src[i]; }
#pragma unroll
      for (int u = 0; u < NA_U; ++u) { int k = tid + u * PT; int i = k < HD_V0 ? k : k - HD_V0 + HD_V1; if (k < NA) lds[i] = va[u]; }
    }
    for (int c = wave; c < HD_CHUNKS; c += PW) dma_chunk(src + HD_V0 + 64 * c + lane, lds + HD_V0 + 64 * c);
  }
  unsigned long long* prof = a.prof ? prof_lds : nullptr;
  if (prof && tid < 16) prof_lds[tid] = 0;
  if (tid < 4) (&glist_n[0][0])[tid] = 0;
  if (tid == 0) conflict_lds = 0;
  if (tid >= 64 && tid < 64 + 4 + NRED) (&work.phish_mask[0])[tid - 64] = 0;
  static_assert(offsetof(StepWork, pend_r) == offsetof(StepWork, phish_mask) + 16, "phish_mask and pend_r are cleared as one run of words");
  if (tid >= 128 && tid < 128 + 5) work.hdirty[tid - 128] = 0;
  __syncthreads();
  EnvState* s = reinterpret_cast<EnvState*>(lds);
  HostDyn* const hd = s->hd;
  if (prof && tid == 0) prof[11] += clock64() - t_begin;
  const bool do_reset = a.autoreset && s->done;
  if (do_reset) {
    dma_wait();
    __syncthreads();
    reset_counter_mode_block<PT, true>(s, hd, cold_e, &work, tid, reset_ws, 0, true, a.steps, a.policy, a.topo);
    if (tid == 0) { a.reward[e] = s->reward; a.done[e] = s->done; }
    __syncthreads();
  } else {
    const int st_now = s->step_count;
    const bool step_ok = step_phase_of(st_now, s->phase_len[0], s->phase_len[1], s->phase_len[2]) >= 0;
    if (tid == 0) {
      Ctx x{s, cold_e, &s->rng, hd, &work, prof};
      x.lg = (LOG && cold_e->evlog.enabled) ? &cold_e->evlog : nullptr;
      x.ext = (LOG && a.ext) ? a.ext + (size_t)e * EXT_PER_ENV : nullptr;
      CC4_TICK0(x);
      (void)step_phase(x, false);
    }
    if (step_ok) {
      Ctx x0p{s, cold_e, nullptr, hd, &work, tid == 0 ? prof : nullptr};
      const int ng = s->n_green;
      if (tid == 0) CC4_TICK(x0p, 0);
      Rng rl;
      rng_fork(&rl, &s->rng, ST_RESET);
      rl.mode = 3;
      rng_begin_step(&rl, (uint32_t)st_now);
      EvLog* const lg = (LOG && cold_e->evlog.enabled) ? &cold_e->evlog : nullptr;
      const ExtAct* const xt = (LOG && a.ext) ? a.ext + (size_t)e * EXT_PER_ENV : nullptr;
      Ctx x0{s, cold_e, &rl, hd, &work, tid == 0 ? prof : nullptr};
      x0.lg = lg; x0.ext = xt;
      constexpr int RW = 2;
      const int ragent = lane * RW + wave;
      const bool is_red = wave < RW && lane < (NRED + RW - 1) / RW && ragent < NRED;
      unsigned long long* ap = (a.prof && is_red) ? a.prof + PROF_SLOTS * (size_t)e + 16 + 8 * ragent : nullptr;
      constexpr int RWX = 4;
      const int xagent = lane * RWX + wave;
      const bool is_redx = wave < RWX && lane < (NRED + RWX - 1) / RWX && xagent < NRED;
      unsigned long long* apx = (a.prof && is_redx) ? a.prof + PROF_SLOTS * (size_t)e + 16 + 8 * xagent : nullptr;
      Ctx xrx{s, cold_e, &rl, hd, &work, nullptr, apx, lg};
      Ctx xr{s, cold_e, &rl, hd, &work, nullptr, ap, lg};
      xrx.ext = xt; xr.ext = xt;

      if (is_red) {
        unsigned long long t0 = ap ? clock64() : 0;
        const int dropped = step_red_policy_tick(xr, ragent);
        if (ap) ap[0] += clock64() - t0;
        if (dropped) atomicSub(&s->n_actions, 1);
      }
      else if (wave == PW - 1 && lane >= 2 && lane < 2 + NBLUE) {
        const int b = lane - 2;
        int32_t act = a.actions ? a.actions[e * NBLUE + b] : -1;
        if (a.rand_out) { act = random_blue_action(a.rand_seed0, a.rand_t, e, b); a.rand_out[e * NBLUE + b] = act; }
        step_blue_submit(x0, b, act);
        step_tick_blue(x0, b);
        step_messages(s, a.msgs ? a.msgs + e * NBLUE * MSG_LEN : nullptr, b);
        { uint32_t c[4]; rng_block(&rl, ST_BLUE_EXE + (uint32_t)b, 0, c); reinterpret_cast<uint4*>(reset_ws)[MAXG + NRED + b] = make_uint4(c[0], c[1], c[2], c[3]); }
      }
      else if (wave == PW - 2 && lane >= 1 && lane <= NRED) {
        uint32_t c[4]; rng_block(&rl, ST_RED_EXE + (uint32_t)(lane - 1), 0, c); reinterpret_cast<uint4*>(reset_ws)[MAXG + lane - 1] = make_uint4(c[0], c[1], c[2], c[3]);
      }
      else if (lane >= 8 && wave >= PW - 2) {
        static_assert((RW <= PW - 2 || RW >= NRED) && MAXG <= 2 * (WAVE - 8), "every green agent has its own lane (8..63) on one of the last two waves, which carry no red agent or one on lane 0: one pass, one ballot per type");
        const int gw = wave - (PW - 2);
        const int g = gw * (WAVE - 8) + (lane - 8);
        if (g < ng) {
          Ctx xg{s, cold_e, &rl, hd, &work, nullptr, nullptr, lg};
          xg.ext = xt;
          step_green_policy(xg, g);
          const int t = work.green_act[g];
          const unsigned long long m0 = __ballot(t == 0), m1 = __ballot(t == 1);
          const unsigned long long below = (1ull << lane) - 1ull;
          if (t < 2) {
            const unsigned long long m = t == 0 ? m0 : m1;
            glist[t][gw][__popcll(m & below)] = (uint8_t)g;
            if ((m & below) == 0) glist_n[t][gw] = __popcll(m);
            uint32_t c[4];
            rng_block(&rl, ST_GREEN_EXE + (uint32_t)g, 0, c);
            reinterpret_cast<uint4*>(reset_ws)[g] = make_uint4(c[0], c[1], c[2], c[3]);
          }
        }
      }
      if (a.prof && lane == 63) a.prof[PROF_SLOTS * (size_t)e + 100 + wave] += clock64() - t_begin;
      dma_wait();
      __syncthreads();
      CC4_TICK(x0, 2);
      if (blue_exec_independent(s)) {
        if (tid == 0) CC4_TICK(x0, 3);
        constexpr int BW = PW;
        const int bagent = lane * BW + wave;
// ... 121 lines not shown
```

cage_challenge_4_amd/csrc/cc4_kernels.h:

```cpp
#pragma once
#include "cc4_args.h"

#ifdef CC4_BOUNDARY_PROF
#define CC4_BP(...) do { if constexpr (HEAD) { __VA_ARGS__; } } while (0)
__shared__ unsigned long long cc4_bp_staged;
#else
#define CC4_BP(...) do {} while (0)
#endif

__device__ __forceinline__ int32_t random_blue_action(uint64_t seed0, uint32_t t, int e, int b) {
  uint32_t c[4] = {t, (uint32_t)b, 0xB10Eu, 0u};
  uint64_t key = seed0 + (uint64_t)e;
  philox4x32_10(c, (uint32_t)key, (uint32_t)(key >> 32));
  uint32_t range = b == 4 ? ACT_LONG : ACT_SHORT;
  return (int32_t)(((uint64_t)c[0] * range) >> 32);
}

template <int NVEC>
__device__ __forceinline__ void stage_in(uint4* __restrict__ lds, const uint4* __restrict__ src, int lane) {
  constexpr int U = NVEC / WAVE < 8 ? (NVEC / WAVE > 0 ? NVEC / WAVE : 1) : 8;
  int i = lane;
  for (; i + (U - 1) * WAVE < NVEC; i += U * WAVE) {
    uint4 v[U];
#pragma unroll
    for (int u = 0; u < U; ++u) v[u] = src[i + u * WAVE];
#pragma unroll
    for (int u = 0; u < U; ++u) lds[i + u * WAVE] = v[u];
  }
  for (; i < NVEC; i += WAVE) lds[i] = src[i];
}
template <int NVEC>
__device__ __forceinline__ void stage_out(uint4* __restrict__ dst, const uint4* __restrict__ lds, int lane) {
  constexpr int U = NVEC / WAVE < 8 ? (NVEC / WAVE > 0 ? NVEC / WAVE : 1) : 8;
  int i = lane;
  for (; i + (U - 1) * WAVE < NVEC; i += U * WAVE) {
    uint4 v[U];
#pragma unroll
    for (int u = 0; u < U; ++u) v[u] = lds[i + u * WAVE];
#pragma unroll
    for (int u = 0; u < U; ++u) dst[i + u * WAVE] = v[u];
  }
  for (; i < NVEC; i += WAVE) dst[i] = lds[i];
}

__device__ __forceinline__ uint8_t pack_obs_byte(const uint8_t* vals, int j) {
  uint32_t b = 0;
#pragma unroll
  for (int k = 0; k < 4; ++k) { const int i = 4 * j + k; if (i < OBS_TOTAL) b |= (uint32_t)(vals[i] & 3u) << (2 * k); }
  return (uint8_t)b;
}

__device__ __forceinline__ void store_packed_row(uint8_t* o8, const uint8_t* vals, int t, int nt) {
  uint32_t* o32 = reinterpret_cast<uint32_t*>(o8);
  for (int w = t; w < OBS_PACKED / 4; w += nt) {
    const uint32_t v = (uint32_t)pack_obs_byte(vals, 4 * w) | ((uint32_t)pack_obs_byte(vals, 4 * w + 1) << 8) |
                       ((uint32_t)pack_obs_byte(vals, 4 * w + 2) << 16) | ((uint32_t)pack_obs_byte(vals, 4 * w + 3) << 24);
    __hip_atomic_store(o32 + w, v, __ATOMIC_RELAXED, __HIP_MEMORY_SCOPE_SYSTEM);
  }
}
__device__ __forceinline__ void pack_row_from_obs(uint8_t* o8, const int32_t* o, int lane) {
  static_assert((OBS_TOTAL * 4) % 8 == 0, "rows of the int32 observation buffer are 8-byte aligned: two values per load");
  if (lane < OBS_PACKED / 4) {
    const uint2* o2 = reinterpret_cast<const uint2*>(o + 16 * lane);
    uint2 w[8];
#pragma unroll
    for (int k = 0; k < 8; ++k) w[k] = (16 * lane + 2 * k < OBS_TOTAL) ? o2[k] : make_uint2(0u, 0u);
    uint32_t v = 0;
#pragma unroll
    for (int k = 0; k < 8; ++k) v |= ((w[k].x & 3u) << (4 * k)) | ((w[k].y & 3u) << (4 * k + 2));
    __hip_atomic_store(reinterpret_cast<uint32_t*>(o8) + lane, v, __ATOMIC_RELAXED, __HIP_MEMORY_SCOPE_SYSTEM);
  }
}
__device__ __forceinline__ void raise_timeout(const XchgArgs& x) {
  __hip_atomic_store(x.timeout, 1u, __ATOMIC_RELAXED, __HIP_MEMORY_SCOPE_SYSTEM);
  __hip_atomic_store(x.timeout_host, 1u, __ATOMIC_RELAXED, __HIP_MEMORY_SCOPE_SYSTEM);
}
__device__ __forceinline__ void xchg_wait_slab(const XchgArgs& x, uint32_t k, uint32_t& seen) {
  if (k < (uint32_t)x.ring || !x.gathered) return;
  const uint32_t need = k - (uint32_t)x.ring + 1u;
  if (seen >= need) return;
  seen = __hip_atomic_load(x.gathered, __ATOMIC_RELAXED, __HIP_MEMORY_SCOPE_SYSTEM);
  if (seen >= need) return;
  if (__hip_atomic_load(x.timeout, __ATOMIC_RELAXED, __HIP_MEMORY_SCOPE_SYSTEM)) return;
  const long long w0 = wall_clock64();
  int naps = 1;
  while ((seen = __hip_atomic_load(x.gathered, __ATOMIC_RELAXED, __HIP_MEMORY_SCOPE_SYSTEM)) < need) {
    for (int i = 0; i < naps; ++i) __builtin_amdgcn_s_sleep(127);
    if (naps < 16) naps <<= 1;
    if (wall_clock64() - w0 > x.wait_ticks || __hip_atomic_load(x.timeout, __ATOMIC_RELAXED, __HIP_MEMORY_SCOPE_SYSTEM)) { raise_timeout(x); return; }
  }
}
__device__ __forceinline__ void xchg_count(const XchgArgs& x, uint32_t k, int group) {
  (void)__hip_atomic_fetch_add(x.gcnt + (size_t)group * (size_t)x.ring + (k % (uint32_t)x.ring), 1u, __ATOMIC_RELAXED, __HIP_MEMORY_SCOPE_AGENT);
}
template <bool WAIT, class StoreRow>
__device__ __forceinline__ void xchg_step_out(const XchgArgs& x, int n, int e, int k, uint32_t& seen, StoreRow store_row) {
  if (threadIdx.x == 0) { if (k > 0) xchg_count(x, (uint32_t)(k - 1), xchg_group32(e)); if (WAIT) xchg_wait_slab(x, (uint32_t)k, seen); }
  store_row(x.slab + ((size_t)(k % x.ring) * (size_t)n + (size_t)e) * OBS_PACKED);
}
__device__ __forceinline__ void xchg_last_out(const XchgArgs& x, int e, int K) {
  if (x.slab && K > 0) {
    asm volatile("s_waitcnt vmcnt(0)" ::: "memory");
    if (threadIdx.x == 0) xchg_count(x, (uint32_t)(K - 1), xchg_group32(e));
  }
}
struct MonitorWatchTab { uint32_t v[(MAXH + 3) / 4]; };
constexpr MonitorWatchTab make_monitor_watch_tab() { MonitorWatchTab t{}; for (int w = 0; w < (MAXH + 3) / 4; ++w) t.v[w] = monitor_watch_mask(w); return t; }
static __device__ const MonitorWatchTab monitor_watch_tab = make_monitor_watch_tab();
__device__ __forceinline__ void monitor_roll_all(EnvState* s, int lane) {
  static_assert((MAXH + 3) / 4 <= WAVE && offsetof(EnvState, hev) % 4 == 0, "one pass of the wave over aligned words");
  if (lane < (MAXH + 3) / 4) {
    uint32_t* const w = reinterpret_cast<uint32_t*>(s->hev) + lane;
    *w = monitor_roll4(*w, monitor_watch_tab.v[lane]);
  }
}
struct ObsFastTab { uint32_t v[OBS_FAST]; };
constexpr ObsFastTab make_obs_fast_tab() {
  ObsFastTab t{};
  for (int v = 0; v < OBS_FAST; ++v) {
    const uint32_t e = obs_fast_entry(v), src = (e >> 10) & 0xFFu;
    const uint32_t off = src < (uint32_t)MAXH ? (uint32_t)offsetof(EnvState, hev) + src : (uint32_t)offsetof(EnvState, msg) + (src - (uint32_t)MAXH);
    t.v[v] = ((e & 0x3FFu) << 2) | (off << 12) | ((e >> 18) << 25);
  }
  return t;
}
static_assert(offsetof(EnvState, hev) + MAXH <= 8192 && offsetof(EnvState, msg) + NBLUE * MSG_LEN <= 8192, "source offsets fit 13 bits");
static_assert((EV_CUR_PROC | EV_OLD_PROC | EV_CUR_CONN | EV_OLD_CONN) < 128 && OBS_TOTAL * 4 <= 4096, "mask and byte position fit their fields");
static __device__ const ObsFastTab obs_fast_tab = make_obs_fast_tab();
template <int nt>
__device__ __forceinline__ void encode_obs_fast(const EnvState* s, int32_t* o, uint8_t* obs_bytes, bool pack, int t, bool msgs_clean = false) {
  constexpr int NV = (OBS_FAST + nt - 1) / nt;
  constexpr int K_MSG = (224 + nt - 1) / nt;
  constexpr bool EXACT = OBS_FAST % nt == 0;
  const uint32_t tt = (uint32_t)t;
  __builtin_assume(tt < (uint32_t)nt);
  uint32_t ent[NV];
#pragma unroll
  for (int k = 0; k < NV; ++k) { const uint32_t v = tt + (uint32_t)(k * nt); ent[k] = (EXACT || v < (uint32_t)OBS_FAST) ? obs_fast_tab.v[v] : 0u; }
  const uint8_t* const row = reinterpret_cast<const uint8_t*>(s);
  char* const ob = reinterpret_cast<char*>(o);
#pragma unroll
  for (int k = 0; k < NV; ++k) {
    const uint32_t v = tt + (uint32_t)(k * nt);
    if (!EXACT && v >= (uint32_t)OBS_FAST) continue;
    if (k >= K_MSG && msgs_clean) continue;
    const uint32_t byte = row[(ent[k] >> 12) & 0x1FFFu];
    const int val = (byte & (ent[k] >> 25)) != 0 ? 1 : 0;
    const uint32_t pos = ent[k] & 0xFFFu;
    *reinterpret_cast<int32_t*>(ob + pos) = val;
    if (pack) obs_bytes[pos >> 2] = (uint8_t)val;
  }
}
__device__ __forceinline__ void encode_obs_slow(const EnvState* s, int32_t* o, uint32_t dirty, int lane) {
  if (!dirty) return;
  auto put = [&](int v) { int i; const int val = env_flat_obs_sorted(s, v, &i); o[i] = val; };
  if ((dirty & OD_BLOCKS) && lane < 63) put(OBS_FAST + lane);
  if (dirty & OD_PHASE) { if (lane < 63) put(OBS_FAST + 63 + lane); if (lane < 5) put(OBS_FAST + 189 + lane); }
  if ((dirty & ~(uint32_t)(OD_BLOCKS | OD_PHASE)) && lane < 63) put(OBS_FAST + 126 + lane);
}
__device__ __forceinline__ void episode_set_seed(EnvState* s, EnvCold* c, uint64_t seed, int rng_mode) {
  if (rng_mode == 0) {
    if (!s->rng_split) c->rng2 = s->rng;
    s->rng_split = 1;
  }
  rng_seed(&s->rng, seed, (uint32_t)rng_mode);
  if (rng_mode == 1) { rng_begin_episode(&s->rng); rng_park(&s->rng); }
}
template <int NT, bool RNG_COPY>
__device__ __forceinline__ void reset_counter_mode_block(EnvState* s, HostDyn* const hd, EnvCold* const cold_e, StepWork* const work, const int t, uint32_t* const ws,
                                                         const uint64_t seed, const bool continue_stream, const int steps, const int policy, const uint32_t topo) {
  reset_zero(s, hd, cold_e, t, NT);
  __syncthreads();
  Rng rr; ResetCarry carry; carry.env_key = 0;
  Ctx xm{s, cold_e, RNG_COPY ? &rr : &s->rng, hd, work};
  if (t == 0) {
    if (RNG_COPY) { rr = s->rng; rr.mode = 1; }
    carry = reset_topology<1>(xm, seed, steps, continue_stream, policy, topo, ws, RNG_COPY, ResetHostLater{});
  }
  __syncthreads();
  Rng rh; rng_fork(&rh, &s->rng, ST_GEN_HOST); rh.mode = 1;
  Ctx xh{s, cold_e, &rh, hd, work};
  if constexpr (NT >= MAXH) { if (t < MAXH) reset_gen_host<1>(xh, t); } else { for (int h = t; h < MAXH; h += NT) reset_gen_host<1>(xh, h); }
  __syncthreads();
  if (t == 0) { reset_pid_serial(xm, reset_used_set(s)); reset_agents(xm); }
  __syncthreads();
  reset_used_clear(s, t, NT);
  __syncthreads();
  if constexpr (NT >= MAXH) { if (t < MAXH) reset_host_sessions(xh, t); } else { for (int h = t; h < MAXH; h += NT) reset_host_sessions(xh, h); }
  __syncthreads();
  if (t == 0) reset_finish(xm, carry, steps, topo, RNG_COPY);
}
```

cage_challenge_4_amd/csrc/cc4_persist.h:

```cpp
#pragma once
#include "cc4_kernels.h"

template <bool LOG> __device__ __forceinline__ void pcg_body(StepArgs a, const int e, const int lane, const bool first = true, const bool last = true);
template <bool LOG, bool PERSIST, bool HEAD> __device__ __forceinline__ void philox1_body(StepArgs a, const int e, const uint32_t rand_t, const uint32_t item_k, const int lane,
                                                                const bool first, const bool last);

__device__ __forceinline__ int cu_slot() {
  const uint32_t hw = __builtin_amdgcn_s_getreg(((16 - 1) << 11) | (0 << 6) | 4);
  const uint32_t xcc = __builtin_amdgcn_s_getreg(((4 - 1) << 11) | (0 << 6) | 20);
  return (int)(((xcc & 7u) << 8) | ((hw >> 8) & 0xFFu));
}
static_assert(MAX_XCD_PARTITIONS == WAVE, "pick_balanced: one lane per partition of the wave's XCD");
__device__ __forceinline__ void rollout_wait_actions(const RunArgs& ra, const XchgArgs& x, int line, int g, uint32_t j) {
  const uint32_t* w = ra.act_ready + (size_t)line * 32 + g;
  if (__hip_atomic_load(w, __ATOMIC_RELAXED, __HIP_MEMORY_SCOPE_SYSTEM) > j) return;
  if (__hip_atomic_load(x.timeout, __ATOMIC_RELAXED, __HIP_MEMORY_SCOPE_SYSTEM)) return;
  const long long w0 = wall_clock64();
  int naps = 1;
  while (__hip_atomic_load(w, __ATOMIC_RELAXED, __HIP_MEMORY_SCOPE_SYSTEM) <= j) {
    for (int i = 0; i < naps; ++i) __builtin_amdgcn_s_sleep(32);
    if (naps < 4) naps <<= 1;
    if (wall_clock64() - w0 > ra.act_wait_ticks || __hip_atomic_load(x.timeout, __ATOMIC_RELAXED, __HIP_MEMORY_SCOPE_SYSTEM)) { raise_timeout(x); return; }
  }
}
__device__ __forceinline__ uint32_t wait_progress(const RunArgs& ra, const XchgArgs& x, int ee, uint32_t k, const bool watchdog, bool& ok) {
  const long long w0 = watchdog ? wall_clock64() : 0;
  uint32_t w;
  ok = true;
  while ((progress_steps(w = __hip_atomic_load(&ra.progress[ee], __ATOMIC_RELAXED, __HIP_MEMORY_SCOPE_AGENT)) - ra.base) < k) {
    if (watchdog && wall_clock64() - w0 > ra.act_wait_ticks) { raise_timeout(x); ok = false; break; }
    __builtin_amdgcn_s_sleep(8);
  }
  return w;
}
__device__ __forceinline__ bool draw_ticket(const RunArgs& ra, int n, int line, int idx, int pg, int& j, int& ee) {
  const uint32_t cnt = ticket_count(n, ra.P, line, idx, pg), total = ticket_total(cnt, ra.runs.nph);
  const uint32_t t = __hip_atomic_fetch_add(ra.ticket + line * TK_STRIDE + idx, 1u, __ATOMIC_RELAXED, __HIP_MEMORY_SCOPE_AGENT);
  if (t + 1u == total) __hip_atomic_store(ra.ticket_next + line * TK_STRIDE + idx, 0u, __ATOMIC_RELAXED, __HIP_MEMORY_SCOPE_AGENT);
  if (t >= total) return false;
  ticket_item(t, cnt, line, idx, pg, ra.P, j, ee);
  return true;
}

template <bool PCG>
__device__ __forceinline__ void persist_step_out(const StepArgs& a, const RunArgs& ra, const XchgArgs& x, const bool rollout, const int lane, const int e, const uint32_t k,
                                                 int& pend_e, uint32_t& pend_k) {
  if constexpr (PCG) {
    if (lane == 0) xchg_count(x, k, part_of(e, ra.G));
  } else {
    if (lane == 0 && pend_e >= 0) xchg_count(x, pend_k, part_of(pend_e, ra.G));
    pack_row_from_obs(x.slab + ((size_t)(k % (uint32_t)x.ring) * (size_t)a.n + (size_t)e) * OBS_PACKED, a.obs + (size_t)e * OBS_TOTAL, lane);
    pend_e = e; pend_k = k;
    if (rollout) {
      asm volatile("s_waitcnt vmcnt(0)" ::: "memory");
      if (lane == 0) xchg_count(x, k, pgroup_slot(e, ra.P, ra.PG));
      pend_e = -1;
    }
  }
}

template <bool PCG, bool ROLLOUT = false, bool XCHG = true, bool PLAN = false, bool HEAD = false>
__device__ __forceinline__ void persist_loop(StepArgs a, RunArgs ra, const XchgArgs x, const PlanArgs pl = PlanArgs{}) {
  static_assert(!HEAD || (!PCG && !ROLLOUT && !XCHG && !PLAN), "the headline build: counter mode, nothing but the steps");
  const int lane = threadIdx.x;
  const int my_slot = cu_slot();
  a.prof = nullptr; a.obs8 = nullptr; a.ext = nullptr;
  uint32_t seen_gathered = 0;
  unsigned long long tl_first = 0, tl_last = 0, tl_items = 0;
  const unsigned long long tl_entry = ra.timeline ? wall_clock64() : 0;
#ifdef CC4_BOUNDARY_PROF
  unsigned long long bp_t = 0, bp_A = 0, bp_B = 0, bp_C = 0, bp_D = 0, bp_n = 0;
#endif
  auto tl_flush = [&]() {
#ifdef CC4_BOUNDARY_PROF
    if (HEAD && ra.timeline && lane == 0) { unsigned long long* t = ra.timeline + 4 * (size_t)blockIdx.x; t[0] = ((tl_last - tl_first) & 0xFFFFFFFFull) | (bp_n << 32) | (1ull << 63); t[1] = (bp_A & 0xFFFFFFFFull) | (bp_B << 32); t[2] = (bp_C & 0xFFFFFFFFull) | (bp_D << 32); t[3] = tl_items | ((unsigned long long)(my_slot + 1) << 32); return; }
#endif
    if (ra.timeline && lane == 0) { unsigned long long* t = ra.timeline + 4 * (size_t)blockIdx.x; t[0] = tl_entry; t[1] = tl_first; t[2] = tl_last; t[3] = tl_items | ((unsigned long long)(my_slot + 1) << 32); } };
  int pend_e = -1; uint32_t pend_k = 0;
  auto flush_pending = [&]() {
    if (XCHG && x.slab && pend_e >= 0) { asm volatile("s_waitcnt vmcnt(0)" ::: "memory"); if (lane == 0) xchg_count(x, pend_k, part_of(pend_e, ra.G)); pend_e = -1; }
  };
  const int my_xcc = my_slot >> 8;
  const int xlo = ra.xcc_lo[my_xcc], xn = ra.xcc_n[my_xcc];
  const int own = ra.slot_part[my_slot] - 1;
  const uint32_t my_id = runner_of(own);
  const bool rollout = ROLLOUT && ra.act_ready;
  if (xn <= 0) { tl_flush(); return; }

  struct Item { int e, k, sh; };
  auto claim = [&](int line, int idx, int pg, Item& it) -> int {
    int j, ee;
    if (!draw_ticket(ra, a.n, line, idx, pg, j, ee)) return 0;
    CC4_BP(const unsigned long long now = wall_clock64(); if (tl_items) bp_B += now - bp_t; bp_t = now);
    int k, len; run_span(ra.runs, j, k, len);
    bool ok;
    const uint32_t w = wait_progress(ra, x, ee, (uint32_t)k, rollout, ok);
    if (!ok) return -1;
    __builtin_amdgcn_fence(__ATOMIC_ACQUIRE, "workgroup");
    CC4_BP(const unsigned long long now = wall_clock64(); if (tl_items) bp_C += now - bp_t; bp_t = now);
    if (XCHG && !rollout && x.slab) xchg_wait_slab(x, (uint32_t)k, seen_gathered);
    const uint32_t last = progress_runner(w);
    it.e = ee; it.k = j; it.sh = (last != RUNNER_NONE && last != my_id) ? 1 : 0;
    return 1;
  };
  auto pick_rollout = [&]() -> Item {
    Item it{-4, 0, 0};
    if (own < 0 || lane != 0) return it;
    const int ne = part_episodes(a.n, ra.P, own);
    const uint32_t* rdy = ra.act_ready + (size_t)own * 32;
    const uint32_t* tkl = ra.ticket + (size_t)own * TK_STRIDE;
    int naps = 1;
    const long long w0 = wall_clock64();
    for (;;) {
      int best_g = -1; uint32_t best_j = 0xFFFFFFFFu; bool left = false;
      for (int g = 0; g < ra.PG; ++g) {
        const int ng = pgroup_episodes(ne, ra.PG, g);
        if (ng <= 0) continue;
        const uint32_t t = __hip_atomic_load(tkl + g, __ATOMIC_RELAXED, __HIP_MEMORY_SCOPE_AGENT);
        if (t >= ticket_total(ng, ra.runs.nph)) continue;
        left = true;
        const uint32_t j = ticket_run(t, ng);
        if (j < best_j && __hip_atomic_load(rdy + g, __ATOMIC_RELAXED, __HIP_MEMORY_SCOPE_SYSTEM) > j) { best_j = j; best_g = g; }
      }
      if (!left) return it;
      if (best_g >= 0) {
        const int got = claim(own, best_g, ra.PG, it);
        if (got == 0) continue;
        if (got > 0) rollout_wait_actions(ra, x, own, best_g, (uint32_t)it.k);
        return it;
      }
      for (int q = 0; q < naps; ++q) __builtin_amdgcn_s_sleep(32);
      if (naps < 4) naps <<= 1;
      if (__hip_atomic_load(x.timeout, __ATOMIC_RELAXED, __HIP_MEMORY_SCOPE_SYSTEM) || wall_clock64() - w0 > ra.act_wait_ticks) {
        raise_timeout(x);
        for (int g = 0; g < ra.PG; ++g) {
          if (pgroup_episodes(ne, ra.PG, g) <= 0) continue;
          const int got = claim(own, g, ra.PG, it);
          if (got > 0) it.sh = 1;
          if (got != 0) return it;
        }
      }
    }
  };
  auto pick_balanced = [&]() -> Item {
    Item it{-5, 0, 0};
    const int q = xlo + lane;
    uint32_t tk = 0xFFFFFFFFu, tot_q = 0;
    if (lane < xn) { tk = __hip_atomic_load(&ra.ticket[q * TK_STRIDE], __ATOMIC_RELAXED, __HIP_MEMORY_SCOPE_AGENT); tot_q = ticket_total(part_episodes(a.n, ra.P, q), ra.runs.nph); }
    const bool has = lane < xn && tk < tot_q;
    uint32_t key = has ? ((tk << 6) | (uint32_t)lane) : 0xFFFFFFFFu;
#pragma unroll
    for (int off = 32; off >= 1; off >>= 1) { const uint32_t k2 = (uint32_t)__shfl_xor((int)key, off); key = k2 < key ? k2 : key; }
    const uint32_t kmin = (uint32_t)__builtin_amdgcn_readfirstlane((int)key);
    if (kmin == 0xFFFFFFFFu) { it.e = -4; return it; }
    int target = (int)(kmin & 63u);
    if (own >= 0) {
      const int ol = own - xlo;
      const uint32_t tk_own = (uint32_t)__builtin_amdgcn_readlane((int)tk, ol);
      const uint32_t tot_own = (uint32_t)__builtin_amdgcn_readlane((int)tot_q, ol);
      if (tk_own < tot_own && tk_own <= (kmin >> 6) + (uint32_t)ra.thr) target = ol;
    }
    if (lane == 0) (void)claim(xlo + target, 0, 1, it);
    return it;
  };
  for (;;) {
    const Item it = rollout ? pick_rollout() : pick_balanced();
    const int e = __builtin_amdgcn_readfirstlane(it.e);
    if (e == -4) { flush_pending(); tl_flush(); return; }
    if (e == -5) continue;
    int run_k0, run_len;
    run_span(ra.runs, __builtin_amdgcn_readfirstlane(it.k), run_k0, run_len);
    if (ra.timeline && !tl_items) tl_first = wall_clock64();
    if (__builtin_amdgcn_readfirstlane(it.sh)) __builtin_amdgcn_fence(__ATOMIC_ACQUIRE, "agent");
    uint32_t item_k = (uint32_t)run_k0;
    uint32_t err_acc = 0;
    for (int q = 0; q < run_len; ++q, ++item_k) {
      if (q > 0) {
        if (XCHG && x.slab) {
          asm volatile("s_waitcnt vmcnt(0)" ::: "memory");
          __syncthreads();
          persist_step_out<PCG>(a, ra, x, rollout, lane, e, item_k - 1u, pend_e, pend_k);
          if (lane == 0) xchg_wait_slab(x, item_k, seen_gathered);
        }
        __syncthreads();
      }
      int lane_i = (int)threadIdx.x;
      asm volatile("" : "+v"(lane_i));
      if (rollout) { a.actions = ra.act + (size_t)(item_k & 1u) * (size_t)a.n * NBLUE; a.rand_out = nullptr; a.act_sys = 1; }
      if constexpr (PLAN) {
        const size_t row = (size_t)item_k * (size_t)a.n;
        a.actions = pl.actions + row * NBLUE; a.msgs = pl.msgs ? pl.msgs + row * (NBLUE * MSG_LEN) : nullptr; a.rand_out = nullptr;
        if (pl.rewards) a.reward = pl.rewards + row;
        if (pl.dones) a.done = pl.dones + row;
        a.obs8 = pl.obs_packed ? pl.obs_packed + row * OBS_PACKED : nullptr;
      }
      if constexpr (PCG) {
        StepArgs b = a;
        b.rand_t = ra.t0 + item_k; b.full_obs = (a.full_obs && item_k == 0) ? 1 : 0;
        if (XCHG && x.slab) b.obs8 = x.slab + (size_t)(item_k % (uint32_t)x.ring) * (size_t)a.n * OBS_PACKED;
        pcg_body<false>(b, e, lane_i, q == 0, q == run_len - 1);
      } else {
        philox1_body<false, true, HEAD>(a, e, ra.t0 + item_k, item_k, lane_i, q == 0, q == run_len - 1);
      }
      if constexpr (PLAN) {
        extern __shared__ uint4 plan_lds[];
        const EnvState* const sp = reinterpret_cast<const EnvState*>(plan_lds);
        if (lane == 0) err_acc |= sp->err | (sp->step_count == 0 ? PLAN_REGEN : 0u);
      }
    }
    --item_k;
    CC4_BP(if (tl_items) { bp_D += cc4_bp_staged - bp_t; ++bp_n; } bp_t = wall_clock64());
    asm volatile("s_waitcnt vmcnt(0)" ::: "memory");
    __builtin_amdgcn_fence(__ATOMIC_RELEASE, "workgroup");
    __syncthreads();
    if (XCHG && x.slab) persist_step_out<PCG>(a, ra, x, rollout, lane, e, item_k, pend_e, pend_k);
    if constexpr (PLAN) {
      if (lane == 0 && err_acc) (void)__hip_atomic_fetch_or(pl.err_or + e, err_acc, __ATOMIC_RELAXED, __HIP_MEMORY_SCOPE_AGENT);
    }
    if (lane == 0) __hip_atomic_store(&ra.progress[e], progress_pack(ra.base + item_k + 1u, my_id), __ATOMIC_RELAXED, __HIP_MEMORY_SCOPE_AGENT);
    if (ra.timeline) { tl_last = wall_clock64(); ++tl_items; }
    CC4_BP(bp_A += tl_last - bp_t; bp_t = tl_last);
  }
}
```

cage_challenge_4_amd/csrc/cc4_philox1_body.h:

```cpp
#pragma once
#include "cc4_kernels.h"

__device__ __forceinline__ void philox1_autoreset(const StepArgs& a, const int e, const int lane, EnvState* s, HostDyn* const hd, EnvCold* const cold_e, StepWork& work) {
    reset_counter_mode_block<WAVE, true>(s, hd, cold_e, &work, lane, a.reset_ws + (size_t)e * RESET_WS_WORDS, 0, true, a.steps, a.policy, a.topo);
    if (lane == 0) { a.reward[e] = s->reward; a.done[e] = s->done; }
    __syncthreads();
}

#ifndef CC4_STOP_IN_FAST
#define CC4_STOP_IN_FAST 0
#endif
#define CC4_STOP_ON (LOG || CC4_STOP_IN_FAST)
#define CC4_STOP(n) do { if (CC4_STOP_ON && a.dbg_stop == (n)) return; } while (0)
template <bool LOG, bool PERSIST, bool HEAD = false>
__device__ __forceinline__ void philox1_body(StepArgs a, const int e, const uint32_t rand_t, const uint32_t item_k, const int lane,
                                             const bool first = true, const bool last = true) {
  static_assert(!HEAD || (PERSIST && !LOG), "the headline build is a fast persistent build");
  if constexpr (HEAD) { a.actions = nullptr; a.msgs = nullptr; a.act_sys = 0; a.obs8 = nullptr; }
  extern __shared__ uint4 lds[];
  __shared__ StepWork work;
  __shared__ unsigned long long prof_lds[LOG ? 16 : 1];
  if constexpr (!LOG) a.prof = nullptr;
  (void)item_k;
  EnvCold* const cold_e = cold_at(a.cold, (size_t)e, cold_row_bytes(a.steps));
  unsigned long long t_begin = a.prof ? clock64() : 0;
  const uint4* src = reinterpret_cast<const uint4*>(a.st + e);
  if (first) stage_in<HOT_VEC>(lds, src, lane);
  for (int i = lane; i < (int)(sizeof(StepWork) / 4); i += WAVE) reinterpret_cast<uint32_t*>(&work)[i] = 0;
  unsigned long long* prof = a.prof ? prof_lds : nullptr;
  if (prof && lane < 16) prof_lds[lane] = 0;
  __syncthreads();
#ifdef CC4_BOUNDARY_PROF
  if constexpr (HEAD) { if (first && lane == 0) cc4_bp_staged = wall_clock64(); }
#endif
  EnvState* s = reinterpret_cast<EnvState*>(lds);
  HostDyn* const hd = a.st[e].hd;
  if (prof && lane == 0) prof[11] += clock64() - t_begin;
  const bool do_reset = a.autoreset && s->done;
  const bool msgs_clean = PERSIST && item_k > 0 && !a.msgs;
  if (do_reset) {
    philox1_autoreset(a, e, lane, s, hd, cold_e, work);
  } else {
    const int st_now = s->step_count;
    const bool step_ok = step_phase_of(st_now, s->phase_len[0], s->phase_len[1], s->phase_len[2]) >= 0;
    if (lane == 0) {
      Ctx x{s, cold_e, &s->rng, hd, &work, prof};
      x.lg = (LOG && cold_e->evlog.enabled) ? &cold_e->evlog : nullptr;
      x.ext = (LOG && a.ext) ? a.ext + (size_t)e * EXT_PER_ENV : nullptr;
      CC4_TICK0(x);
      (void)step_phase(x, false);
    }
    if (step_ok) {
      CC4_STOP(1);
      const int ng = s->n_green;
      Rng rl;
      rng_fork(&rl, &s->rng, ST_RESET);
      rl.mode = 3;
      rng_begin_step(&rl, (uint32_t)st_now);
      EvLog* const lg = (LOG && cold_e->evlog.enabled) ? &cold_e->evlog : nullptr;
      const ExtAct* const xt = (LOG && a.ext) ? a.ext + (size_t)e * EXT_PER_ENV : nullptr;
      Ctx x0{s, cold_e, &rl, hd, &work, lane == 0 ? prof : nullptr};
      x0.lg = lg; x0.ext = xt;
      if (lane == 0) CC4_TICK(x0, 0);
      enum : int { BK_GPOL = 0, BK_GEXE = 16, BK_RPOL = 32, BK_REXE = 38, BK_BEXE = 44, BK_BRAND = 49, BK_END = 54 };
      uint32_t bank[4];
      {
        uint32_t st = 0;
        if (lane < BK_GEXE) st = ST_GREEN_POL + (uint32_t)(WAVE + lane - BK_GPOL);
        else if (lane < BK_REXE) st = ST_RED_POL + (uint32_t)(lane - BK_RPOL);
        else if (lane < BK_BEXE) st = ST_RED_EXE + (uint32_t)(lane - BK_REXE);
        else if (lane < BK_BRAND) st = ST_BLUE_EXE + (uint32_t)(lane - BK_BEXE);
        bank[0] = 0u; bank[1] = st; bank[2] = (uint32_t)rl.inc_lo; bank[3] = (uint32_t)rl.inc_hi;
        uint32_t k0 = (uint32_t)rl.s_lo, k1 = (uint32_t)(rl.s_lo >> 32);
        if ((HEAD || a.rand_out) && lane >= BK_BRAND && lane < BK_END) {
          const uint64_t key = a.rand_seed0 + (uint64_t)e;
          bank[0] = rand_t; bank[1] = (uint32_t)(lane - BK_BRAND); bank[2] = 0xB10Eu; bank[3] = 0u; k0 = (uint32_t)key; k1 = (uint32_t)(key >> 32);
        }
        philox4x32_10(bank, k0, k1, true);
      }
      auto bank_fetch = [&](int shift, uint32_t out[4]) {
        const int addr = ((lane + shift) & (WAVE - 1)) << 2;
#pragma unroll
        for (int k = 0; k < 4; ++k) out[k] = (uint32_t)__builtin_amdgcn_ds_bpermute(addr, (int)bank[k]);
      };
      CC4_STOP(2);
      const bool is_red = lane < NRED;
      unsigned long long* ap = (a.prof && is_red) ? a.prof + PROF_SLOTS * (size_t)e + 16 + 8 * lane : nullptr;
      Ctx xr{s, cold_e, &rl, hd, &work, nullptr, ap, lg};
      Ctx xg{s, cold_e, &rl, hd, &work, nullptr, nullptr, lg};
      xr.ext = xt; xg.ext = xt;
      uint32_t pre_rp[4];
      bank_fetch(BK_RPOL, pre_rp);
      const uint32_t brand = (uint32_t)__builtin_amdgcn_ds_bpermute(((lane + BK_BRAND - 8) & (WAVE - 1)) << 2, (int)bank[0]);
      if (is_red) {
        unsigned long long t0 = ap ? clock64() : 0;
        const int dropped = step_red_policy_tick(xr, lane, false, pre_rp);
        if (ap) ap[0] += clock64() - t0;
        if (dropped) atomicSub(&s->n_actions, 1);
      } else if (lane >= 8 && lane < 8 + NBLUE && !(CC4_STOP_ON && a.dbg_stop == 3)) {
        const int b = lane - 8;
        int32_t act = !a.actions ? -1 : a.act_sys ? __hip_atomic_load(a.actions + e * NBLUE + b, __ATOMIC_RELAXED, __HIP_MEMORY_SCOPE_SYSTEM) : a.actions[e * NBLUE + b];
        if (HEAD || a.rand_out) { act = (int32_t)(((uint64_t)brand * (uint32_t)(b == 4 ? ACT_LONG : ACT_SHORT)) >> 32); a.rand_out[e * NBLUE + b] = act; }
        step_blue_submit(xg, b, act);
        step_tick_blue(xg, b);
        if (!msgs_clean) step_messages(s, a.msgs ? a.msgs + e * NBLUE * MSG_LEN : nullptr, b);
      }
      if (!(CC4_STOP_ON && (a.dbg_stop == 3 || a.dbg_stop == 4))) {
        if (lane < ng) step_green_policy(xg, lane);
        if (lane + WAVE < ng) step_green_policy(xg, lane + WAVE, bank);
      }
      __syncthreads();
      CC4_TICK(x0, 2);
      CC4_STOP(3); CC4_STOP(4); CC4_STOP(5);
      {
        const bool indep = blue_exec_independent(s);
        if (lane == 0) CC4_TICK(x0, 3);
        uint32_t c[4];
        bank_fetch(BK_BEXE, c);
        Ctx xb = xg;
        if (!indep) xb.prof = x0.prof;
        const int rounds = indep ? 1 : 2 * NBLUE;
#pragma nounroll
        for (int i = 0; i < rounds; ++i) {
          int b = lane;
// ... 128 lines not shown
```

cage_challenge_4_amd/csrc/cc4_rng.h:

```cpp
#pragma once
#include <stdint.h>
#include <stddef.h>

#if defined(__HIPCC__)
#define CC4_HD __host__ __device__ __forceinline__
#define CC4_UNROLL _Pragma("unroll")
#else
#define CC4_HD inline
#define CC4_UNROLL
#endif

namespace cc4 {

CC4_HD uint64_t mulhi64(uint64_t a, uint64_t b) {
#if defined(__HIP_DEVICE_COMPILE__)
  return __umul64hi(a, b);
#else
  return (uint64_t)(((unsigned __int128)a * b) >> 64);
#endif
}

struct Rng {
  uint64_t s_hi, s_lo;
  uint64_t inc_hi, inc_lo;
  uint32_t has32;
  uint32_t u32;
  uint32_t mode;
  uint32_t ndraw;
  uint64_t buf64;
  uint32_t has64, pad;
};

enum : uint32_t { ST_RESET = 0, ST_BLUE_EXE = 0x100, ST_GREEN_POL = 0x200, ST_GREEN_EXE = 0x300, ST_GREEN_PHISH = 0x400,
                  ST_RED_POL = 0x500, ST_RED_EXE = 0x600, ST_RED_RSC = 0x700,
                  ST_GEN_HOST = 0x800, ST_GEN_REDRAW = 0x900, ST_GEN_SESS = 0xA00,
                  ST_BLUE_POL = 0xB00  };

CC4_HD uint32_t ss_hashmix(uint32_t value, uint32_t* hash_const) {
  value ^= *hash_const;
  *hash_const *= 0x931e8875u;
  value *= *hash_const;
  value ^= value >> 16;
  return value;
}
CC4_HD uint32_t ss_mix(uint32_t x, uint32_t y) {
  uint32_t r = 0xca01f9ddu * x - 0x4973f715u * y;
  r ^= r >> 16;
  return r;
}
CC4_HD void seed_sequence_state(uint64_t seed, uint64_t out[4]) {
  uint32_t ent[2];
  int n_ent = 1;
  ent[0] = (uint32_t)seed;
  ent[1] = (uint32_t)(seed >> 32);
  if (ent[1] != 0) n_ent = 2;
  uint32_t pool[4];
  uint32_t hc = 0x43b0d7e5u;
  for (int i = 0; i < 4; ++i) pool[i] = ss_hashmix(i < n_ent ? ent[i] : 0u, &hc);
  for (int i_src = 0; i_src < 4; ++i_src)
    for (int i_dst = 0; i_dst < 4; ++i_dst)
      if (i_src != i_dst) pool[i_dst] = ss_mix(pool[i_dst], ss_hashmix(pool[i_src], &hc));
  uint32_t hb = 0x8b51f9ddu;
  uint32_t w[8];
  for (int i = 0; i < 8; ++i) {
    uint32_t d = pool[i & 3];
    d ^= hb;
    hb *= 0x58f38dedu;
    d *= hb;
    d ^= d >> 16;
    w[i] = d;
  }
  for (int i = 0; i < 4; ++i) out[i] = (uint64_t)w[2 * i] | ((uint64_t)w[2 * i + 1] << 32);
}

#define CC4_PCG_MULT_HI 0x2360ED051FC65DA4ull
#define CC4_PCG_MULT_LO 0x4385DF649FCCF645ull

CC4_HD void pcg_step(Rng* r) {
  uint64_t lo = r->s_lo * CC4_PCG_MULT_LO;
  uint64_t hi = mulhi64(r->s_lo, CC4_PCG_MULT_LO) + r->s_hi * CC4_PCG_MULT_LO + r->s_lo * CC4_PCG_MULT_HI;
  uint64_t nlo = lo + r->inc_lo;
  hi += r->inc_hi + (nlo < lo ? 1ull : 0ull);
  r->s_lo = nlo;
  r->s_hi = hi;
}

CC4_HD uint32_t philox_xor3(uint32_t a, uint32_t b, uint32_t c, bool vec) {
#if defined(__HIP_DEVICE_COMPILE__)
  if (vec) return __builtin_amdgcn_bitop3_b32(a, b, c, 0x96);
#endif
  (void)vec;
  return a ^ b ^ c;
}
CC4_HD void philox4x32_10(uint32_t c[4], uint32_t k0, uint32_t k1, bool vec = false) {
  for (int i = 0; i < 10; ++i) {
    uint64_t p0 = (uint64_t)0xD2511F53u * c[0];
    uint64_t p1 = (uint64_t)0xCD9E8D57u * c[2];
    uint32_t n0 = philox_xor3((uint32_t)(p1 >> 32), c[1], k0, vec);
    uint32_t n1 = (uint32_t)p1;
    uint32_t n2 = philox_xor3((uint32_t)(p0 >> 32), c[3], k1, vec);
    uint32_t n3 = (uint32_t)p0;
    c[0] = n0; c[1] = n1; c[2] = n2; c[3] = n3;
    k0 += 0x9E3779B9u;
    k1 += 0xBB67AE85u;
  }
}

CC4_HD void rng_seed(Rng* r, uint64_t seed, uint32_t mode) {
  r->has32 = 0; r->u32 = 0; r->mode = mode; r->ndraw = 0; r->buf64 = 0; r->has64 = 0; r->pad = 0;
  if (mode == 0) {
    uint64_t v[4];
    seed_sequence_state(seed, v);
    r->inc_hi = (v[2] << 1) | (v[3] >> 63);
    r->inc_lo = (v[3] << 1) | 1ull;
    r->s_hi = 0; r->s_lo = 0;
    pcg_step(r);
    uint64_t lo = r->s_lo + v[1];
    r->s_hi = r->s_hi + v[0] + (lo < r->s_lo ? 1ull : 0ull);
    r->s_lo = lo;
    pcg_step(r);
  } else {
    r->s_lo = seed;
    r->s_hi = 0;
    r->inc_hi = 0;
    r->inc_lo = 0;
  }
}

CC4_HD void rng_begin_step(Rng* r, uint32_t step) {
  if (r->mode & 1u) { r->inc_lo = (uint64_t)step; r->s_hi = 0; r->has32 = 0; r->has64 = 0; r->ndraw = 0; }
}
CC4_HD void rng_set_stream(Rng* r, uint32_t id) {
  if (r->mode & 1u) { r->ndraw = id; r->s_hi = 0; r->has32 = 0; r->has64 = 0; }
}
CC4_HD void rng_park(Rng* r) {
  if (r->mode & 1u) { r->s_hi = 0; r->has32 = 0; r->u32 = 0; r->ndraw = 0; r->has64 = 0; r->buf64 = 0; r->pad = 0; }
}
CC4_HD void rng_fork(Rng* r, const Rng* parent, uint32_t id) {
  *r = *parent;
  rng_set_stream(r, id);
}
CC4_HD void rng_begin_episode(Rng* r) {
  if (r->mode & 1u) { r->inc_hi++; r->inc_lo = 0xFFFFFFFFull; r->s_hi = 0; r->has32 = 0; r->has64 = 0; r->ndraw = ST_RESET; }
}

CC4_HD uint32_t philox_next32(Rng* r) {
  if (r->has64 == 0) {
    uint32_t c[4] = {(uint32_t)r->s_hi, r->ndraw, (uint32_t)r->inc_lo, (uint32_t)r->inc_hi};
    philox4x32_10(c, (uint32_t)r->s_lo, (uint32_t)(r->s_lo >> 32), r->mode == 3u);
    r->s_hi++;
    r->u32 = c[0]; r->pad = c[1]; r->buf64 = (uint64_t)c[2] | ((uint64_t)c[3] << 32); r->has64 = 4;
  }
  const uint32_t out = r->u32;
  r->u32 = r->pad; r->pad = (uint32_t)r->buf64; r->buf64 >>= 32; r->has64--;
  return out;
}
CC4_HD uint64_t rng_next64(Rng* r) {
  if (r->mode & 1u) { const uint64_t lo = philox_next32(r); return lo | ((uint64_t)philox_next32(r) << 32); }
  r->ndraw++;
  pcg_step(r);
  uint64_t x = r->s_hi ^ r->s_lo;
  uint32_t rot = (uint32_t)(r->s_hi >> 58);
  return (x >> rot) | (x << ((64u - rot) & 63u));
}

CC4_HD void rng_block(const Rng* r, uint32_t stream, uint32_t ctr, uint32_t c[4]) {
  c[0] = ctr; c[1] = stream; c[2] = (uint32_t)r->inc_lo; c[3] = (uint32_t)r->inc_hi;
  philox4x32_10(c, (uint32_t)r->s_lo, (uint32_t)(r->s_lo >> 32), r->mode == 3u);
}
CC4_HD void rng_preload(Rng* r, const uint32_t c[4]) {
  r->u32 = c[0]; r->pad = c[1]; r->buf64 = (uint64_t)c[2] | ((uint64_t)c[3] << 32); r->has64 = 4; r->has32 = 0; r->s_hi = 1;
}
CC4_HD uint32_t rng_next32(Rng* r) {
  if (r->mode & 1u) return philox_next32(r);
  if (r->has32) { r->has32 = 0; return r->u32; }
  uint64_t n = rng_next64(r);
  r->has32 = 1;
  r->u32 = (uint32_t)(n >> 32);
  return (uint32_t)n;
}

CC4_HD uint32_t rng_next32(Rng* r);
CC4_HD double rng_random(Rng* r) {
  if (r->mode & 1u) return (double)rng_next32(r) * (1.0 / 4294967296.0);
  return (double)(rng_next64(r) >> 11) * (1.0 / 9007199254740992.0);
}

CC4_HD bool rng_random_lt(Rng* r, double t) {
  if (r->mode & 1u) {
    const uint32_t k = rng_next32(r);
    const double s = t * 4294967296.0;
    if (!(s > 0.0)) return false;
    if (s >= 4294967296.0) return true;
    const uint64_t f = (uint64_t)s;
    return (uint64_t)k < f + ((double)f < s ? 1u : 0u);
  }
  return rng_random(r) < t;
}
CC4_HD bool rng_random_le(Rng* r, double t) {
  if (r->mode & 1u) {
    const uint32_t k = rng_next32(r);
    const double s = t * 4294967296.0;
    if (!(s >= 0.0)) return false;
    if (s >= 4294967296.0) return true;
    return (uint64_t)k <= (uint64_t)s;
  }
  return rng_random(r) <= t;
}
CC4_HD int rng_random_quarter(Rng* r) {
  if (r->mode & 1u) return (int)(rng_next32(r) >> 30);
  return (int)(rng_random(r) * 4.0);
}

CC4_HD uint32_t rng_below(Rng* r, uint32_t n) {
  if (n <= 1) return 0;
  uint32_t rng_excl = n;
  uint64_t m = (uint64_t)rng_next32(r) * rng_excl;
  uint32_t leftover = (uint32_t)m;
  if (leftover < rng_excl) {
    uint32_t threshold = (uint32_t)((0xFFFFFFFFu - (n - 1)) % rng_excl);
    while (leftover < threshold) {
      m = (uint64_t)rng_next32(r) * rng_excl;
      leftover = (uint32_t)m;
    }
  }
  return (uint32_t)(m >> 32);
}
CC4_HD int32_t rng_range(Rng* r, int32_t lo, int32_t hi) { return lo + (int32_t)rng_below(r, (uint32_t)(hi - lo)); }

CC4_HD uint32_t rng_interval(Rng* r, uint32_t max) {
  if (max == 0) return 0;
  uint32_t mask = max;
// ... 11 lines not shown
```

Measured before the change: 1.686 billion.

## Parallelize autoreset: prefill philox bank, split pid settle, vectorize zeroing

The environment regeneration path is restructured. Philox blocks for the reset stream are precomputed in parallel across lanes into a bank held in idle red-agent memory, and the serial topology and agent draws read from it. The pid pass is split into a parallel gather, a short serial settle and a parallel write-back. Reset zeroing now uses 16-byte stores, and the per-env reset workspace is dropped. This aims to shorten the single-lane serial section of each autoreset, at the cost of extra synchronisation, bank fill and clear work, and a dependence on scratch space inside the red agents.

```diff
diff --git a/cage_challenge_4_amd/csrc/cc4_api.hip b/cage_challenge_4_amd/csrc/cc4_api.hip
--- a/cage_challenge_4_amd/csrc/cc4_api.hip
+++ b/cage_challenge_4_amd/csrc/cc4_api.hip
@@ -38,7 +38,7 @@
   a.n = h->cfg.num_envs; a.autoreset = h->cfg.autoreset; a.steps = h->cfg.steps; a.rng_mode = h->cfg.rng_mode;
   a.policy = policy_bits(h->cfg);
   a.topo = (uint32_t)h->cfg.topology_seed;
-  a.reset_ws = h->d_reset_ws;
+  a.green_win = h->d_green_win;
   return a;
 }
 RunArgs run_args(const cc4_handle* h, int k, uint32_t t0, bool head) {
@@ -296,7 +296,7 @@
   size_t n = (size_t)cfg->num_envs;
   h->cold_row = cold_row_bytes(cfg->steps);
   if (dev_alloc(h, &h->d_state, n * sizeof(EnvState)) || dev_alloc(h, &h->d_cold, n * h->cold_row)) return -1;
-  if (dev_alloc(h, &h->d_reset_ws, cfg->rng_mode == 1 ? n * RESET_WS_WORDS * sizeof(uint32_t) : n * 128 * sizeof(uint64_t))) return -1;
+  if (cfg->rng_mode != 1 && dev_alloc(h, &h->d_green_win, n * 128 * sizeof(uint64_t))) return -1;
   h->in_bytes = n * NBLUE * sizeof(int32_t) + n * NBLUE * MSG_LEN;
   h->small_io = cfg->num_envs <= cc4_handle::SMALL_IO_ENVS;
   if (const char* v = getenv("CC4_SMALL_IO")) h->small_io = h->small_io && atoi(v) != 0;
diff --git a/cage_challenge_4_amd/csrc/cc4_api_debug.hip b/cage_challenge_4_amd/csrc/cc4_api_debug.hip
--- a/cage_challenge_4_amd/csrc/cc4_api_debug.hip
+++ b/cage_challenge_4_amd/csrc/cc4_api_debug.hip
@@ -21,6 +21,28 @@
                       "(first item's start to last item's end, mean %.1f us); kernel (events) %.1f us\n", k, rs.SA, rs.nA, rs.SB, rs.nB, rs.nph, nw, sn, items,
                       sA / sn / 100.0, sB / sn / 100.0, sC / sn / 100.0, sD / sn / 100.0, (sA + sB + sC + sD) / sn / 100.0, per[0], per[m / 2], per[m * 9 / 10], per[m - 1],
                       100.0 * (sA + sB + sC + sD) / busy_ticks, busy_ticks / nw / 100.0, ms * 1000.0);
+      return 0;
+    }
+  }
+#endif
+#ifdef CC4_REGEN_PROF
+  { double sp[RP_PHASES] = {0}, sn = 0, items = 0; int nw = 0; bool head = false; std::vector<double> per;
+    for (int w = 0; w < h->run_grid; ++w) { const unsigned long long* t = &tl[4 * (size_t)w]; if (!(t[0] >> 63)) continue; head = true;
+      const double n = (double)(t[2] >> 42); items += (double)(uint32_t)t[3]; if (n <= 0) continue; ++nw; sn += n;
+      double all = 0;
+      for (int i = 0; i < RP_PHASES; ++i) { const double v = (double)((t[i / 3] >> (21 * (i % 3))) & 0x1FFFFFull); sp[i] += v; all += v; }
+      per.push_back(all / n / 100.0); }
+    if (head) {
+      float ms = 0.f; if (timed) (void)hipEventElapsedTime(&ms, h->evs[0], h->evs[1]);
+      std::sort(per.begin(), per.end());
+      const size_t m = per.size();
+      double all = 0; for (double v : sp) all += v;
+      if (m) fprintf(stderr, "[cc4 regen] k=%d: %d waves regenerated, %.0f regenerations (%.0f items); per regeneration, mean us of wave time: zero %.2f, topology %.2f, hosts %.2f, pid settle %.2f, "
+                      "pid write-back / set clear %.2f, agents %.2f, sessions + backup %.2f, finish %.2f, all %.2f; per wave all: min %.2f / median %.2f / 90%% %.2f / max %.2f us; kernel (events) %.1f us; the regenerations are %.2f %% of the launch's wave time (%d waves x kernel time)\n",
+                      k, nw, sn, items, sp[RP_ZERO] / sn / 100.0, sp[RP_TOPOLOGY] / sn / 100.0, sp[RP_GEN_HOST] / sn / 100.0, sp[RP_PID_SETTLE] / sn / 100.0, sp[RP_PID_WRITEBACK] / sn / 100.0,
+                      sp[RP_AGENTS] / sn / 100.0, sp[RP_SESSIONS] / sn / 100.0, sp[RP_FINISH] / sn / 100.0, all / sn / 100.0, per[0], per[m / 2], per[m * 9 / 10], per[m - 1], ms * 1000.0,
+                      ms > 0.f ? 100.0 * all / ((double)h->run_grid * ms * 1e5) : 0.0, h->run_grid);
+      else fprintf(stderr, "[cc4 regen] k=%d: no regeneration in this call (%.0f items); kernel (events) %.1f us\n", k, items, ms * 1000.0);
       return 0;
     }
   }
diff --git a/cage_challenge_4_amd/csrc/cc4_args.h b/cage_challenge_4_amd/csrc/cc4_args.h
--- a/cage_challenge_4_amd/csrc/cc4_args.h
+++ b/cage_challenge_4_amd/csrc/cc4_args.h
@@ -30,6 +30,9 @@
 #define CC4_PHILOX_BIG_MINW 7
 #endif
 
+enum : int { RP_ZERO = 0, RP_TOPOLOGY, RP_GEN_HOST, RP_PID_SETTLE, RP_PID_WRITEBACK, RP_AGENTS, RP_SESSIONS, RP_FINISH, RP_PHASES };
+struct RegenProf { unsigned long long t; uint32_t p[RP_PHASES]; uint32_t n; };
+
 struct StepArgs {
   EnvState* st; EnvCold* cold;
   const int32_t* actions; const uint8_t* msgs;
@@ -41,7 +44,7 @@
   int full_obs;
   uint32_t topo;
   unsigned long long* prof;
-  uint32_t* reset_ws;
+  uint64_t* green_win;
   const ExtAct* ext;
   int e0;
   int act_sys;
diff --git a/cage_challenge_4_amd/csrc/cc4_engine.h b/cage_challenge_4_amd/csrc/cc4_engine.h
--- a/cage_challenge_4_amd/csrc/cc4_engine.h
+++ b/cage_challenge_4_amd/csrc/cc4_engine.h
@@ -630,16 +630,20 @@
 }
 
 struct ResetCarry { uint64_t env_key; };
-enum : int { RESET_WS_SEEN = 0, RESET_WS_DUP = 288, RESET_WS_HOSTS = 576, RESET_WS_WORDS = 584 };
+enum : int { RESET_WS_WORDS = 584 };
 
 CC4_HD void reset_zero(EnvState* s, HostDyn* hd, EnvCold* c, int t, int nt) {
   static_assert(offsetof(EnvState, rng) == 0, "the generator leads the row");
   uint32_t* w = (uint32_t*)s;
   for (size_t i = sizeof(Rng) / 4 + (size_t)t; i < offsetof(EnvState, hd) / 4; i += (size_t)nt) w[i] = i == PA_WORD ? w[i] & PA_WORD_MASK : 0;
-  uint32_t* hw = (uint32_t*)hd;
-  for (size_t i = (size_t)t; i < sizeof(HostDyn) * MAXH / 4; i += (size_t)nt) hw[i] = 0;
-  uint32_t* b = (uint32_t*)c->hs;
-  for (size_t i = (size_t)t; i < sizeof(c->hs) / 4; i += (size_t)nt) b[i] = 0;
+  static_assert(sizeof(HostDyn) * MAXH % 16 == 0 && alignof(HostDyn) >= 16 && alignof(EnvCold) >= 16 && offsetof(EnvCold, hs) == 0 && sizeof(EnvCold::hs) % 16 == 8,
+                "whole vectors of the host table; whole vectors and one 8-byte word of the backup images");
+  struct alignas(16) Vec16 { uint32_t w[4]; };
+  Vec16* hw = (Vec16*)hd;
+  for (size_t i = (size_t)t; i < sizeof(HostDyn) * MAXH / 16; i += (size_t)nt) hw[i] = Vec16{{0u, 0u, 0u, 0u}};
+  Vec16* b = (Vec16*)c->hs;
+  for (size_t i = (size_t)t; i < sizeof(c->hs) / 16; i += (size_t)nt) b[i] = Vec16{{0u, 0u, 0u, 0u}};
+  if (t == 0) *(uint64_t*)((char*)c->hs + sizeof(c->hs) - 8) = 0;
 }
 static_assert(sizeof(RSess) * RS_POOL >= 4 * 282, "the idle session pool holds the 9000-bit pid set of the generation");
 CC4_HD uint32_t* reset_used_set(EnvState* s) { return reinterpret_cast<uint32_t*>(s->spool); }
@@ -692,7 +696,7 @@
   ResetCarry k; k.env_key = x.r->s_lo;
   if (RNG_MODE == 1 && topo_seed) x.r->s_lo = (uint64_t)topo_seed;
   reset_mission_phases(s, steps);
-  if (RNG_MODE == 1) for (int i = 0; i < RESET_WS_WORDS; ++i) ws[i] = 0;
+  (void)ws;
   {
     uint32_t* avail = x.w->scratch;
     for (int i = 0; i < 8; ++i) avail[i] = 0xFFFFFFFFu;
@@ -721,43 +725,91 @@
     for (int i = 0; i < ns; ++i) place(h_make(sn, 11 + i), last_set(ips, 8));
     s->n_users[sn] = (uint8_t)nu; s->n_servers[sn] = (uint8_t)ns;
   }
-  if (RNG_MODE == 1 && rng_is_copy) s->rng = *x.r;
+  if (RNG_MODE == 1 && rng_is_copy) { s->rng = *x.r; s->rng.mode = (uint32_t)RNG_MODE; }
   return k;
 }
-CC4_HD void reset_pid_serial(Ctx x, uint32_t* used) {
-  EnvState* s = x.s;
+enum : int { PC_PER_HOST = 5, PC_MOVED = 0x8000 };
+static_assert(sizeof(RedAgent) * NRED >= 2 * PC_PER_HOST * MAXH && offsetof(EnvState, red) % 2 == 0, "the idle red agents hold the candidates of the pid pass");
+CC4_HD uint16_t* reset_pid_cand(EnvState* s) { return reinterpret_cast<uint16_t*>(s->red); }
+CC4_HD void reset_pid_gather(Ctx x, int h, uint16_t* cand) {
+  if (!bit_get(x.s->exists, h) || h_is_router(h)) return;
+  const HostDyn& st = x.hd[h];
+  const int sub = h_subnet(h);
+  uint16_t* const c = cand + PC_PER_HOST * h;
+  c[0] = st.svcs[0].pid;
+  if (sub == S_OZA || sub == S_OZB) c[1] = st.svcs[1].pid;
+  c[2] = st.procs[5].pid; c[3] = st.procs[6].pid; c[4] = st.svcs[6].pid;
+}
+CC4_HD void reset_pid_settle(const Rng* main, uint16_t* cand, uint32_t* used) {
   for (int h = 0; h < MAXH; ++h) {
-    if (!bit_get(s->exists, h) || h_is_router(h)) continue;
-    HostDyn& st = x.hd[h];
-    const int n = hd_nsvc(st);
-    const int sub = h_subnet(h);
-    const int nfix = (sub == S_OZA || sub == S_OZB) ? 2 : 1;
+    uint16_t* const c = cand + PC_PER_HOST * h;
+    static_assert(PC_PER_HOST == 5, "four candidates in one 64-bit word, the fifth beside it");
+    const uint64_t lo = (uint64_t)c[0] | (uint64_t)c[1] << 16 | (uint64_t)c[2] << 32 | (uint64_t)c[3] << 48;
+    const uint32_t hi = c[4];
+    if (!(lo | hi)) continue;
     Rng t; bool forked = false;
-    auto settle = [&](int v0, bool* moved) {
+    CC4_NOUNROLL
+    for (int k = 0; k < PC_PER_HOST; ++k) {
+      const int v0 = k < 4 ? (int)((lo >> (16 * k)) & 0xFFFFu) : (int)hi;
+      if (!v0) continue;
       int v = v0 - 1000;
-      *moved = false;
+      bool moved = false;
       while (bit_get(used, v)) {
-        if (!forked) { rng_fork(&t, x.r, ST_GEN_REDRAW + (uint32_t)h); forked = true; }
+        if (!forked) { rng_fork(&t, main, ST_GEN_REDRAW + (uint32_t)h); forked = true; }
         v = (int)rng_below(&t, 9000);
-        *moved = true;
+        moved = true;
       }
       bit_set(used, v);
-      return v + 1000;
-    };
-    for (int i = 0; i < nfix; ++i) {
-      bool moved;
-      const int v = settle(st.svcs[i].pid, &moved);
-      if (moved) { st.svcs[i].pid = (uint16_t)v; st.procs[i].pid = (uint16_t)v; }
-    }
-    for (int k = 0; k < 3; ++k) {
-      const int kind = k == 0 ? K_APACHE : (k == 1 ? K_MYSQL : K_SMTP);
-      const int v0 = k == 0 ? st.procs[5].pid : (k == 1 ? st.procs[6].pid : st.svcs[6].pid);
-      bool moved;
-      const int v = settle(v0, &moved);
-      if (moved) for (int i = nfix; i < n; ++i) if (st.svcs[i].kind == kind) { st.svcs[i].pid = (uint16_t)v; st.procs[i].pid = (uint16_t)v; }
-    }
-    st.procs[5].pid = 0; st.procs[6].pid = 0; st.svcs[6].pid = 0;
-  }
+      if (moved) c[k] = (uint16_t)((v + 1000) | PC_MOVED);
+    }
+  }
+}
+CC4_HD void reset_pid_writeback(Ctx x, int h, uint16_t* cand) {
+  if (!bit_get(x.s->exists, h) || h_is_router(h)) return;
+  HostDyn& st = x.hd[h];
+  uint16_t* const c = cand + PC_PER_HOST * h;
+  const int n = hd_nsvc(st);
+  const int sub = h_subnet(h);
+  const int nfix = (sub == S_OZA || sub == S_OZB) ? 2 : 1;
+  for (int i = 0; i < nfix; ++i)
+    if (c[i] & PC_MOVED) { const uint16_t v = (uint16_t)(c[i] & ~PC_MOVED); st.svcs[i].pid = v; st.procs[i].pid = v; }
+  for (int k = 0; k < 3; ++k) {
+    if (!(c[2 + k] & PC_MOVED)) continue;
+    const int kind = k == 0 ? K_APACHE : (k == 1 ? K_MYSQL : K_SMTP);
+    const uint16_t v = (uint16_t)(c[2 + k] & ~PC_MOVED);
+    for (int i = nfix; i < n; ++i) if (st.svcs[i].kind == kind) { st.svcs[i].pid = v; st.procs[i].pid = v; }
+  }
+  st.procs[5].pid = 0; st.procs[6].pid = 0; st.svcs[6].pid = 0;
+  for (int k = 0; k < PC_PER_HOST; ++k) c[k] = 0;
+}
+enum : int { RESET_BANK_BLOCKS = 2 * (int)RNG_BANK_RUN, RESET_BANK_AGENT = 3 };
+static_assert(offsetof(RedAgent, h) >= 16 * RNG_BANK_RUN && sizeof(RedAgent) % 4 == 0 && RESET_BANK_AGENT + 2 <= NRED &&
+              2 * PC_PER_HOST * MAXH <= RESET_BANK_AGENT * sizeof(RedAgent), "two runs of the bank in front of two agents' headers, behind the pid candidates");
+CC4_HD uint32_t* reset_bank(EnvState* s) { return reinterpret_cast<uint32_t*>(&s->red[RESET_BANK_AGENT]); }
+enum : uint32_t { RESET_BANK_HOP = (uint32_t)(sizeof(RedAgent) / 4) - 4u * RNG_BANK_RUN };
+CC4_HD void reset_main_words(Rng* m, const Rng* row, uint32_t topo_seed) {
+  *m = *row; m->mode = 1;
+  rng_begin_episode(m);
+  if (topo_seed) m->s_lo = (uint64_t)topo_seed;
+}
+CC4_HD void reset_bank_fill(EnvState* s, uint32_t topo_seed, int t, int nt, bool vec) {
+  Rng m; reset_main_words(&m, &s->rng, topo_seed);
+  if (vec) m.mode = 3;
+  uint32_t* const bank = reset_bank(s);
+  for (int i = t; i < RESET_BANK_BLOCKS; i += nt) {
+    uint32_t c[4]; rng_block(&m, ST_RESET, (uint32_t)i, c);
+    uint32_t* const w = bank + rng_bank_slot((uint32_t)i, RESET_BANK_HOP);
+    w[0] = c[0]; w[1] = c[1]; w[2] = c[2]; w[3] = c[3];
+  }
+}
+CC4_HD void reset_bank_attach(RngBanked* rr, EnvState* s, bool banked) {
+  *static_cast<Rng*>(rr) = s->rng;
+  rr->mode = banked ? (1u | RNG_BANKED) : 1u;
+  rr->bank = reset_bank(s); rr->bank_n = banked ? (uint32_t)RESET_BANK_BLOCKS : 0u; rr->bank_hop = RESET_BANK_HOP;
+}
+CC4_HD void reset_bank_clear(EnvState* s, int t, int nt) {
+  uint32_t* const bank = reset_bank(s);
+  for (int i = t; i < RESET_BANK_BLOCKS; i += nt) { uint32_t* const w = bank + rng_bank_slot((uint32_t)i, RESET_BANK_HOP); w[0] = 0; w[1] = 0; w[2] = 0; w[3] = 0; }
 }
 CC4_HD void reset_agents(Ctx x) {
   EnvState* s = x.s;
@@ -850,7 +902,7 @@
   s->n_actions = NBLUE + s->n_green + NRED;
   x.c->rwd = RewardRec{};
   if (topo_seed) x.r->s_lo = k.env_key;
-  if (rng_is_copy) s->rng = *x.r;
+  if (rng_is_copy) { s->rng = *x.r; s->rng.mode = s->rng_mode; }
   rng_park(&s->rng);
 }
 CC4_HD void env_reset_counter_mode(Ctx x, uint64_t seed, int steps, bool continue_stream, int policy, uint32_t topo_seed, uint32_t* ws,
@@ -860,9 +912,10 @@
   {
     Rng t; rng_fork(&t, x.r, ST_GEN_HOST);
     Ctx xh = x; xh.r = &t;
-    for (int h = 0; h < MAXH; ++h) reset_gen_host<1>(xh, h);
-  }
-  reset_pid_serial(x, reset_used_set(x.s));
+    for (int h = 0; h < MAXH; ++h) { reset_gen_host<1>(xh, h); reset_pid_gather(xh, h, reset_pid_cand(x.s)); }
+  }
+  reset_pid_settle(x.r, reset_pid_cand(x.s), reset_used_set(x.s));
+  for (int h = 0; h < MAXH; ++h) reset_pid_writeback(x, h, reset_pid_cand(x.s));
   reset_used_clear(x.s, 0, 1);
   reset_agents(x);
   {
diff --git a/cage_challenge_4_amd/csrc/cc4_host.h b/cage_challenge_4_amd/csrc/cc4_host.h
--- a/cage_challenge_4_amd/csrc/cc4_host.h
+++ b/cage_challenge_4_amd/csrc/cc4_host.h
@@ -73,7 +73,7 @@
   bool main_ahead = false;
   unsigned long long* d_prof = nullptr;
   int dbg_stop = 0;
-  uint32_t* d_reset_ws = nullptr;
+  uint64_t* d_green_win = nullptr;
   uint8_t* d_unpacked = nullptr;
   int evlog_on = 0;
   uint32_t* d_run = nullptr;
diff --git a/cage_challenge_4_amd/csrc/cc4_k_misc.hip b/cage_challenge_4_amd/csrc/cc4_k_misc.hip
--- a/cage_challenge_4_amd/csrc/cc4_k_misc.hip
+++ b/cage_challenge_4_amd/csrc/cc4_k_misc.hip
@@ -39,8 +39,7 @@
   for (int i = lane; i < (int)(sizeof(StepWork) / 4); i += WAVE) reinterpret_cast<uint32_t*>(&work)[i] = 0;
   __syncthreads();
   if (a.rng_mode == 1) {
-    __shared__ uint32_t ws[RESET_WS_WORDS];
-    reset_counter_mode_block<WAVE, false>(s, hd, cold_e, &work, lane, ws, a.seeds ? a.seeds[e] : 0, a.seeds == nullptr, a.steps, a.policy, a.topo);
+    reset_counter_mode_block<WAVE, false>(s, hd, cold_e, &work, lane, nullptr, a.seeds ? a.seeds[e] : 0, a.seeds == nullptr, a.steps, a.policy, a.topo);
     __syncthreads();
   } else if (lane == 0) {
     Ctx x{s, cold_e, &s->rng, hd, &work};
diff --git a/cage_challenge_4_amd/csrc/cc4_k_pcg.hip b/cage_challenge_4_amd/csrc/cc4_k_pcg.hip
--- a/cage_challenge_4_amd/csrc/cc4_k_pcg.hip
+++ b/cage_challenge_4_amd/csrc/cc4_k_pcg.hip
@@ -297,7 +297,7 @@
 template <bool LOG>
 __device__ __forceinline__ void pcg_body(StepArgs a, const int e, const int lane, const bool first, const bool last) {
   extern __shared__ uint4 lds[];
-  uint64_t* const win_mem = reinterpret_cast<uint64_t*>(a.reset_ws) + (size_t)e * GW_OUT;
+  uint64_t* const win_mem = a.green_win + (size_t)e * GW_OUT;
   if constexpr (!LOG) a.prof = nullptr;
   __shared__ int ok_lds;
   __shared__ StepWork work;
diff --git a/cage_challenge_4_amd/csrc/cc4_k_philox4.hip b/cage_challenge_4_amd/csrc/cc4_k_philox4.hip
--- a/cage_challenge_4_amd/csrc/cc4_k_philox4.hip
+++ b/cage_challenge_4_amd/csrc/cc4_k_philox4.hip
@@ -73,7 +73,7 @@
   if (do_reset) {
     dma_wait();
     __syncthreads();
-    reset_counter_mode_block<PT, true>(s, hd, cold_e, &work, tid, reset_ws, 0, true, a.steps, a.policy, a.topo);
+    reset_counter_mode_block<PT, true>(s, hd, cold_e, &work, tid, nullptr, 0, true, a.steps, a.policy, a.topo);
     if (tid == 0) { a.reward[e] = s->reward; a.done[e] = s->done; }
     __syncthreads();
   } else {
diff --git a/cage_challenge_4_amd/csrc/cc4_kernels.h b/cage_challenge_4_amd/csrc/cc4_kernels.h
--- a/cage_challenge_4_amd/csrc/cc4_kernels.h
+++ b/cage_challenge_4_amd/csrc/cc4_kernels.h
@@ -6,6 +6,13 @@
 __shared__ unsigned long long cc4_bp_staged;
 #else
 #define CC4_BP(...) do {} while (0)
+#endif
+#ifdef CC4_REGEN_PROF
+#define CC4_RP_BEGIN(rp) do { if (rp) (rp)->t = wall_clock64(); } while (0)
+#define CC4_RP(rp, i) do { if (rp) { const unsigned long long now_ = wall_clock64(); (rp)->p[i] += (uint32_t)(now_ - (rp)->t); (rp)->t = now_; } } while (0)
+#else
+#define CC4_RP_BEGIN(rp) do { (void)(rp); } while (0)
+#define CC4_RP(rp, i) do { (void)(rp); } while (0)
 #endif
 
 __device__ __forceinline__ int32_t random_blue_action(uint64_t seed0, uint32_t t, int e, int b) {
@@ -168,25 +175,41 @@
 }
 template <int NT, bool RNG_COPY>
 __device__ __forceinline__ void reset_counter_mode_block(EnvState* s, HostDyn* const hd, EnvCold* const cold_e, StepWork* const work, const int t, uint32_t* const ws,
-                                                         const uint64_t seed, const bool continue_stream, const int steps, const int policy, const uint32_t topo) {
+                                                         const uint64_t seed, const bool continue_stream, const int steps, const int policy, const uint32_t topo,
+                                                         RegenProf* const rp = nullptr) {
+  CC4_RP_BEGIN(rp);
   reset_zero(s, hd, cold_e, t, NT);
   __syncthreads();
-  Rng rr; ResetCarry carry; carry.env_key = 0;
-  Ctx xm{s, cold_e, RNG_COPY ? &rr : &s->rng, hd, work};
+  CC4_RP(rp, RP_ZERO);
+  const bool banked = RNG_COPY && continue_stream;
+  if (banked) { reset_bank_fill(s, topo, t, NT, true); __syncthreads(); }
+  RngBanked rr; ResetCarry carry; carry.env_key = 0;
+  Ctx xm{s, cold_e, RNG_COPY ? static_cast<Rng*>(&rr) : &s->rng, hd, work};
   if (t == 0) {
-    if (RNG_COPY) { rr = s->rng; rr.mode = 1; }
+    if (RNG_COPY) reset_bank_attach(&rr, s, banked);
     carry = reset_topology<1>(xm, seed, steps, continue_stream, policy, topo, ws, RNG_COPY, ResetHostLater{});
   }
   __syncthreads();
+  CC4_RP(rp, RP_TOPOLOGY);
   Rng rh; rng_fork(&rh, &s->rng, ST_GEN_HOST); rh.mode = 1;
   Ctx xh{s, cold_e, &rh, hd, work};
-  if constexpr (NT >= MAXH) { if (t < MAXH) reset_gen_host<1>(xh, t); } else { for (int h = t; h < MAXH; h += NT) reset_gen_host<1>(xh, h); }
-  __syncthreads();
-  if (t == 0) { reset_pid_serial(xm, reset_used_set(s)); reset_agents(xm); }
-  __syncthreads();
+  uint16_t* const cand = reset_pid_cand(s);
+  for (int h = t; h < MAXH; h += NT) { reset_gen_host<1>(xh, h); reset_pid_gather(xh, h, cand); }
+  __syncthreads();
+  CC4_RP(rp, RP_GEN_HOST);
+  if (t == 0) reset_pid_settle(&s->rng, cand, reset_used_set(s));
+  __syncthreads();
+  CC4_RP(rp, RP_PID_SETTLE);
+  for (int h = t; h < MAXH; h += NT) reset_pid_writeback(xh, h, cand);
   reset_used_clear(s, t, NT);
   __syncthreads();
+  CC4_RP(rp, RP_PID_WRITEBACK);
+  if (t == 0) { reset_agents(xm); if (RNG_COPY) rr.mode = 1; }
+  __syncthreads();
+  CC4_RP(rp, RP_AGENTS);
+  if (banked) reset_bank_clear(s, t, NT);
   if constexpr (NT >= MAXH) { if (t < MAXH) reset_host_sessions(xh, t); } else { for (int h = t; h < MAXH; h += NT) reset_host_sessions(xh, h); }
   __syncthreads();
+  CC4_RP(rp, RP_SESSIONS);
   if (t == 0) reset_finish(xm, carry, steps, topo, RNG_COPY);
 }
diff --git a/cage_challenge_4_amd/csrc/cc4_persist.h b/cage_challenge_4_amd/csrc/cc4_persist.h
--- a/cage_challenge_4_amd/csrc/cc4_persist.h
+++ b/cage_challenge_4_amd/csrc/cc4_persist.h
@@ -71,7 +71,17 @@
 #ifdef CC4_BOUNDARY_PROF
   unsigned long long bp_t = 0, bp_A = 0, bp_B = 0, bp_C = 0, bp_D = 0, bp_n = 0;
 #endif
+#ifdef CC4_REGEN_PROF
+  RegenProf rgp{};
+  RegenProf* const rgp_p = HEAD ? &rgp : nullptr;
+#else
+  RegenProf* const rgp_p = nullptr;
+#endif
   auto tl_flush = [&]() {
+#ifdef CC4_REGEN_PROF
+    if (HEAD && ra.timeline && lane == 0) { unsigned long long* t = ra.timeline + 4 * (size_t)blockIdx.x; auto f = [&](int i) { return (unsigned long long)(rgp.p[i] & 0x1FFFFFu); };
+      t[0] = f(0) | f(1) << 21 | f(2) << 42 | (1ull << 63); t[1] = f(3) | f(4) << 21 | f(5) << 42; t[2] = f(6) | f(7) << 21 | (unsigned long long)rgp.n << 42; t[3] = tl_items | ((unsigned long long)(my_slot + 1) << 32); return; }
+#endif
 #ifdef CC4_BOUNDARY_PROF
     if (HEAD && ra.timeline && lane == 0) { unsigned long long* t = ra.timeline + 4 * (size_t)blockIdx.x; t[0] = ((tl_last - tl_first) & 0xFFFFFFFFull) | (bp_n << 32) | (1ull << 63); t[1] = (bp_A & 0xFFFFFFFFull) | (bp_B << 32); t[2] = (bp_C & 0xFFFFFFFFull) | (bp_D << 32); t[3] = tl_items | ((unsigned long long)(my_slot + 1) << 32); return; }
 #endif
@@ -200,7 +210,7 @@
         if (XCHG && x.slab) b.obs8 = x.slab + (size_t)(item_k % (uint32_t)x.ring) * (size_t)a.n * OBS_PACKED;
         pcg_body<false>(b, e, lane_i, q == 0, q == run_len - 1);
       } else {
-        philox1_body<false, true, HEAD>(a, e, ra.t0 + item_k, item_k, lane_i, q == 0, q == run_len - 1);
+        philox1_body<false, true, HEAD>(a, e, ra.t0 + item_k, item_k, lane_i, q == 0, q == run_len - 1, rgp_p);
       }
       if constexpr (PLAN) {
         extern __shared__ uint4 plan_lds[];
diff --git a/cage_challenge_4_amd/csrc/cc4_philox1_body.h b/cage_challenge_4_amd/csrc/cc4_philox1_body.h
--- a/cage_challenge_4_amd/csrc/cc4_philox1_body.h
+++ b/cage_challenge_4_amd/csrc/cc4_philox1_body.h
@@ -1,10 +1,14 @@
 #pragma once
 #include "cc4_kernels.h"
 
-__device__ __forceinline__ void philox1_autoreset(const StepArgs& a, const int e, const int lane, EnvState* s, HostDyn* const hd, EnvCold* const cold_e, StepWork& work) {
-    reset_counter_mode_block<WAVE, true>(s, hd, cold_e, &work, lane, a.reset_ws + (size_t)e * RESET_WS_WORDS, 0, true, a.steps, a.policy, a.topo);
+__device__ __forceinline__ void philox1_autoreset(const StepArgs& a, const int e, const int lane, EnvState* s, HostDyn* const hd, EnvCold* const cold_e, StepWork& work, RegenProf* const rp) {
+    reset_counter_mode_block<WAVE, true>(s, hd, cold_e, &work, lane, nullptr, 0, true, a.steps, a.policy, a.topo, rp);
     if (lane == 0) { a.reward[e] = s->reward; a.done[e] = s->done; }
     __syncthreads();
+    CC4_RP(rp, RP_FINISH);
+#ifdef CC4_REGEN_PROF
+    if (rp) ++rp->n;
+#endif
 }
 
 #ifndef CC4_STOP_IN_FAST
@@ -14,7 +18,7 @@
 #define CC4_STOP(n) do { if (CC4_STOP_ON && a.dbg_stop == (n)) return; } while (0)
 template <bool LOG, bool PERSIST, bool HEAD = false>
 __device__ __forceinline__ void philox1_body(StepArgs a, const int e, const uint32_t rand_t, const uint32_t item_k, const int lane,
-                                             const bool first = true, const bool last = true) {
+                                             const bool first = true, const bool last = true, RegenProf* const rp = nullptr) {
   static_assert(!HEAD || (PERSIST && !LOG), "the headline build is a fast persistent build");
   if constexpr (HEAD) { a.actions = nullptr; a.msgs = nullptr; a.act_sys = 0; a.obs8 = nullptr; }
   extern __shared__ uint4 lds[];
@@ -39,7 +43,7 @@
   const bool do_reset = a.autoreset && s->done;
   const bool msgs_clean = PERSIST && item_k > 0 && !a.msgs;
   if (do_reset) {
-    philox1_autoreset(a, e, lane, s, hd, cold_e, work);
+    philox1_autoreset(a, e, lane, s, hd, cold_e, work, rp);
   } else {
     const int st_now = s->step_count;
     const bool step_ok = step_phase_of(st_now, s->phase_len[0], s->phase_len[1], s->phase_len[2]) >= 0;
diff --git a/cage_challenge_4_amd/csrc/cc4_rng.h b/cage_challenge_4_amd/csrc/cc4_rng.h
--- a/cage_challenge_4_amd/csrc/cc4_rng.h
+++ b/cage_challenge_4_amd/csrc/cc4_rng.h
@@ -5,9 +5,11 @@
 #if defined(__HIPCC__)
 #define CC4_HD __host__ __device__ __forceinline__
 #define CC4_UNROLL _Pragma("unroll")
+#define CC4_NOUNROLL _Pragma("nounroll")
 #else
 #define CC4_HD inline
 #define CC4_UNROLL
+#define CC4_NOUNROLL
 #endif
 
 namespace cc4 {
@@ -144,10 +146,19 @@
   if (r->mode & 1u) { r->inc_hi++; r->inc_lo = 0xFFFFFFFFull; r->s_hi = 0; r->has32 = 0; r->has64 = 0; r->ndraw = ST_RESET; }
 }
 
+enum : uint32_t { RNG_BANKED = 4u, RNG_BANK_RUN = 32u };
+struct RngBanked : Rng { const uint32_t* bank; uint32_t bank_n, bank_hop; };
+CC4_HD uint32_t rng_bank_slot(uint32_t i, uint32_t hop) { return 4u * i + (i / RNG_BANK_RUN) * hop; }
 CC4_HD uint32_t philox_next32(Rng* r) {
   if (r->has64 == 0) {
     uint32_t c[4] = {(uint32_t)r->s_hi, r->ndraw, (uint32_t)r->inc_lo, (uint32_t)r->inc_hi};
-    philox4x32_10(c, (uint32_t)r->s_lo, (uint32_t)(r->s_lo >> 32), r->mode == 3u);
+    const RngBanked* const b = (r->mode & RNG_BANKED) ? static_cast<const RngBanked*>(r) : nullptr;
+    if (b && c[0] < b->bank_n) {
+      const uint32_t* const w = b->bank + rng_bank_slot(c[0], b->bank_hop);
+      c[0] = w[0]; c[1] = w[1]; c[2] = w[2]; c[3] = w[3];
+    } else {
+      philox4x32_10(c, (uint32_t)r->s_lo, (uint32_t)(r->s_lo >> 32), r->mode == 3u);
+    }
     r->s_hi++;
     r->u32 = c[0]; r->pad = c[1]; r->buf64 = (uint64_t)c[2] | ((uint64_t)c[3] << 32); r->has64 = 4;
   }
```

Result: no change. 1.691 billion (median of 6 runs) (+0.3%).
